# zhaodong-liu/GRAM

Measured on AMD Instinct MI355X. Metric: users/sec @ beam=20 top-20 gen, Beauty T5-base; Recall@5 parity, higher is better.
Workload: dtype f16x3

## Files before the change

### gram_amd/_lib.py

```python
from __future__ import annotations

import ctypes as C
import os

_HERE = os.path.dirname(os.path.abspath(__file__))
LIB_PATH = os.environ.get("GRAM_LIB") or os.path.join(_HERE, "csrc", "libgram_hip.so")

GRAM_MAX_BEAMS = 64
GRAM_MAX_DEC_LEN = 64
GRAM_MAX_PASSAGE_LEN = 128
GRAM_MAX_LONG_PASSAGE_LEN = 512
GRAM_MAX_FUSED_LEN = 4096
GRAM_MAX_LONG_FUSED_LEN = 16384
GRAM_KEY_BITS_LONG_WORDS, GRAM_KEY_BITS_LONG_STRIDE = 512, 528
EPI_BF16, EPI_BF16_RELU, EPI_F32_ADD, EPI_F32, EPI_KV_BANK = range(5)
K_GEMM, K_ENC_ATTN, K_CROSS_ATTN, K_DEC_SELF_ATTN, K_ROWOPS, K_LSE, K_BEAM = range(7)
E_ARG, E_WORKSPACE, E_BEAM, E_NONFINITE = -1, -2, -3, -4
ABI_VERSION = 7
GRAM_MAX_USER_ITEMS = 4096
ITEMS_EXCLUDE, ITEMS_ALLOW = 0, 1
MAX_PIECES = 2
SPLIT_NPROD = (0, 1, 3)


def interleave(pieces):
    p, rows, cols = pieces.shape
    assert p == 2 and cols % 32 == 0
    return pieces.view(2, rows, cols // 32, 32).permute(1, 2, 0, 3).reshape(rows, 2 * cols).contiguous()


def deinterleave(x):
    rows, c2 = x.shape
    return x.view(rows, c2 // 64, 2, 32).permute(2, 0, 1, 3).reshape(2, rows, c2 // 2).contiguous()


STAGES = ("enc_attn", "enc_ffn", "bank_k", "bank_v", "dec_self", "dec_cross", "dec_ffn", "lm_head")

vp = C.c_void_p
i32 = C.c_int32
i64 = C.c_int64
f32 = C.c_float


class KVBank(C.Structure):
    _fields_ = [("k", vp), ("vt", vp), ("n_layers", i32), ("B", i32), ("H", i32), ("S", i32), ("passage_map", vp), ("N", i32),
                ("L", i32)]


class Trie(C.Structure):
    _fields_ = [("child_off", vp), ("child_tok", vp), ("child_node", vp), ("n_nodes", i32), ("n_edges", i32),
                ("max_fanout", i32), ("min_seq_len", i32)]


class LiveRows(C.Structure):
    _fields_ = [("rows", vp), ("rowpos", vp), ("users", vp), ("tokens", vp), ("counts", vp)]


class BeamState(C.Structure):
    _fields_ = [("B", i32), ("K", i32), ("Tmax", i32), ("length_penalty", f32), ("eos", i32), ("pad", i32),
                ("tokens", vp), ("node", vp), ("beam_scores", vp), ("seq", vp), ("anc", vp), ("done", vp),
                ("n_hyps", vp), ("hyp_score", vp), ("worst", vp), ("hyp_len", vp), ("hyp_tok", vp), ("error", vp),
                ("cand_logits", vp), ("cand_logits_users", i32), ("cand_logits_stride", i64)]


class Split(C.Structure):
    _fields_ = [("pieces", i32), ("c_interleaved", i32), ("c_pstride", i64), ("bank_pstride", i64), ("out_scale", f32)]


class NormFusion(C.Structure):
    _fields_ = [("xb_out", vp), ("ss_out", vp), ("ss_in", vp), ("nblk_in", i32), ("d", i32), ("eps", f32), ("quarter", i32),
                ("xs_in", vp), ("xs_out", vp)]


class Compaction(C.Structure):
    _fields_ = [("n_active", i32), ("passage_map", vp), ("ids", vp), ("mask", vp),
                ("n_cached", i32), ("cache_L", i32), ("cache_x", vp), ("cache_slot", vp)]


class UserItems(C.Structure):
    _fields_ = [("leaf_lo", vp), ("leaf_hi", vp), ("ranks", vp), ("count", vp), ("stride", i32), ("mode", i32)]


class XattnOut(C.Structure):
    _fields_ = [("probs", vp), ("layer_probs", vp), ("token_scores", vp), ("passage_scores", vp)]


class TrieRows(C.Structure):
    _fields_ = [("tokens", vp), ("pos", vp), ("anc", vp), ("row_node", vp), ("node_row", vp), ("node_tok", vp), ("node_leaf", vp),
                ("Q", i32), ("Tq", i32), ("n_nodes", i32), ("n_leaves", i32)]


class ModelDesc(C.Structure):
    _fields_ = [
        ("vocab", i32), ("d_model", i32), ("d_ff", i32), ("n_heads", i32), ("n_enc_layers", i32),
        ("n_dec_layers", i32), ("max_passages", i32), ("tie_word_embeddings", i32),
        ("use_position_embedding", i32), ("fold_norm", i32), ("eps", f32),
        ("embed_f32", vp), ("lm_head_bf16", vp), ("pos_emb_f32", vp), ("enc_bias_f32", vp), ("dec_bias_f32", vp),
        ("enc_final_ln", vp), ("dec_final_ln", vp),
        ("enc_ln1", C.POINTER(vp)), ("enc_wqkv", C.POINTER(vp)), ("enc_wo", C.POINTER(vp)),
        ("enc_ln2", C.POINTER(vp)), ("enc_wi", C.POINTER(vp)), ("enc_wo2", C.POINTER(vp)),
        ("dec_ln1", C.POINTER(vp)), ("dec_wqkv", C.POINTER(vp)), ("dec_wo", C.POINTER(vp)),
        ("dec_ln2", C.POINTER(vp)), ("dec_wq_x", C.POINTER(vp)), ("dec_wo_x", C.POINTER(vp)),
        ("dec_ln3", C.POINTER(vp)), ("dec_wi", C.POINTER(vp)), ("dec_wo2", C.POINTER(vp)),
        ("dec_wkv_x_all", vp),
        ("pieces", i32), ("lm_head_f32", vp), ("w_scales", C.POINTER(f32)),
    ]


SIGNATURES = {
    "gram_abi_version": (C.c_int, []),
    "gram_piece_format": (C.c_int, []),
    "gram_gemm_bf16": (C.c_int, [vp, vp, vp, C.c_int, C.c_int, C.c_int, C.c_int, C.c_int, C.c_int, C.POINTER(KVBank), vp]),
    "gram_gemm_bf16_ex": (C.c_int, [vp, vp, vp, C.c_int, C.c_int, C.c_int, C.c_int, C.c_int, C.c_int, C.POINTER(KVBank), C.POINTER(NormFusion), vp]),
    "gram_row_rscale": (C.c_int, [vp, vp, C.c_int, C.c_int, C.c_int, f32, vp]),
    "gram_row_rscale_xs": (C.c_int, [vp, vp, vp, vp, C.c_int, C.c_int, C.c_int, f32, vp]),
    "gram_embed_ex_xs": (C.c_int, [vp, vp, C.c_int, vp, vp, vp, vp, C.c_int, C.c_int, C.c_int, C.c_int, vp]),
    "gram_embed_ex": (C.c_int, [vp, vp, C.c_int, vp, vp, vp, C.c_int, C.c_int, C.c_int, vp]),
    "gram_gemm_bf16_lse": (C.c_int, [vp, vp, vp, vp, C.c_int, C.c_int, C.c_int, C.c_int, C.c_int, vp]),
    "gram_lse_combine": (C.c_int, [vp, vp, C.c_int, C.c_int, vp]),
    "gram_embed_i64": (C.c_int, [vp, vp, vp, C.c_int, C.c_int, vp]),
    "gram_embed_i32": (C.c_int, [vp, vp, vp, C.c_int, C.c_int, vp]),
    "gram_rmsnorm_bf16": (C.c_int, [vp, vp, vp, C.c_int, C.c_int, f32, f32, vp, C.c_int, C.c_int, vp]),
    "gram_enc_self_attn": (C.c_int, [vp, vp, vp, vp, C.c_int, C.c_int, C.c_int, vp]),
    "gram_cross_attn_decode": (C.c_int, [vp, vp, vp, vp, vp, C.c_int, C.c_int, C.c_int, C.c_int, vp]),
    "gram_dec_self_attn": (C.c_int, [vp, vp, vp, vp, vp, vp, C.c_int, C.c_int, C.c_int, C.c_int, vp]),
    "gram_row_lse": (C.c_int, [vp, vp, C.c_int, C.c_int, vp]),
    "gram_beam_init": (C.c_int, [C.POINTER(BeamState), C.POINTER(Trie), C.c_int, vp]),
    "gram_beam_step": (C.c_int, [C.POINTER(BeamState), C.POINTER(Trie), vp, vp, C.c_int, C.c_int, C.c_int, vp]),
    "gram_beam_step_sparse": (C.c_int, [C.POINTER(BeamState), C.POINTER(Trie), vp, vp, C.c_int, vp, C.c_int, C.c_int, C.c_int, vp]),
    "gram_greedy_step": (C.c_int, [C.POINTER(BeamState), C.POINTER(Trie), vp, C.c_int, C.c_int, vp]),
    "gram_greedy_finalize": (C.c_int, [C.POINTER(BeamState), C.c_int, vp, vp, vp]),
    "gram_beam_finalize": (C.c_int, [C.POINTER(BeamState), C.c_int, C.c_int, vp, vp, vp, vp]),
    "gram_trie_item_index": (C.c_int, [C.POINTER(Trie), vp, vp, C.c_int, C.c_int, vp, vp]),
    "gram_model_create": (vp, [C.POINTER(ModelDesc)]),
    "gram_model_destroy": (None, [vp]),
    "gram_iota_i32": (C.c_int, [vp, C.c_int, vp]),
    "gram_token_tables_bytes": (i64, [vp]),
    "gram_token_tables_workspace_bytes": (i64, [vp]),
    "gram_model_build_token_tables": (C.c_int, [vp, vp, i64, vp, i64, vp]),
    "gram_workspace_bytes": (i64, [vp, C.c_int, C.c_int, C.c_int, C.c_int, C.c_int]),
    "gram_workspace_encoder_x_offset": (i64, [vp, C.c_int, C.c_int, C.c_int, C.c_int, C.c_int]),
    "gram_encode_fused": (C.c_int, [vp, vp, vp, C.c_int, C.c_int, C.c_int, vp, i64, C.c_int, C.c_int, vp, vp]),
# ... 20 lines not shown
                                              C.POINTER(UserItems), vp]),
    "gram_beam_step_sparse_split_items": (C.c_int, [C.POINTER(BeamState), C.POINTER(Trie), vp, vp, C.c_int, vp, C.c_int, C.c_int, C.c_int,
                                                    vp, C.c_int, C.POINTER(UserItems), vp]),
    "gram_greedy_step_items": (C.c_int, [C.POINTER(BeamState), C.POINTER(Trie), vp, C.c_int, C.c_int, C.POINTER(UserItems), vp]),
    "gram_generate_items": (C.c_int, [vp, vp, vp, C.c_int, C.c_int, C.c_int, C.c_int, C.c_int, C.c_int, f32, C.POINTER(Trie),
                                      C.POINTER(Compaction), C.POINTER(UserItems), vp, i64, vp, vp, C.POINTER(i32), vp]),
    "gram_encode_passages": (C.c_int, [vp, vp, vp, C.c_int, C.c_int, vp, i64, vp, vp]),
    "gram_gather_passage_x": (C.c_int, [vp, vp, vp, C.c_int, C.c_int, C.c_int, C.c_int, vp]),
    "gram_live_rows": (C.c_int, [C.POINTER(BeamState), C.POINTER(Trie), C.POINTER(LiveRows), vp]),
    "gram_dec_self_attn_live": (C.c_int, [vp, vp, vp, vp, vp, vp, C.c_int, C.c_int, vp, C.c_int, C.c_int, C.c_int, vp]),
    "gram_cross_attn_decode_live": (C.c_int, [vp, vp, vp, vp, vp, C.c_int, vp, vp, C.c_int, C.c_int, C.c_int, vp]),
    "gram_beam_step_sparse_live": (C.c_int, [C.POINTER(BeamState), C.POINTER(Trie), vp, vp, C.c_int, vp, C.c_int, C.c_int, vp, vp]),
    "gram_gemm_bf16_split": (C.c_int, [vp, vp, vp, C.c_int, C.c_int, C.c_int, C.c_int, C.c_int, C.c_int, C.POINTER(KVBank),
                                       C.POINTER(NormFusion), C.POINTER(Split), vp]),
    "gram_gemm_bf16_lse_split": (C.c_int, [vp, vp, vp, vp, C.c_int, C.c_int, C.c_int, C.c_int, C.c_int, C.POINTER(Split), vp]),
    "gram_embed_ex_split": (C.c_int, [vp, vp, C.c_int, vp, vp, vp, C.c_int, C.c_int, C.c_int, C.c_int, vp]),
    "gram_rmsnorm_bf16_split": (C.c_int, [vp, vp, vp, C.c_int, C.c_int, f32, f32, vp, C.c_int, C.c_int, vp, C.c_int, vp]),
    "gram_enc_self_attn_split": (C.c_int, [vp, vp, vp, vp, C.c_int, C.c_int, C.c_int, C.c_int, i64, vp]),
    "gram_cross_attn_decode_split": (C.c_int, [vp, vp, vp, vp, vp, C.c_int, C.c_int, C.c_int, C.c_int, vp, vp, C.c_int, i64, i64, vp, vp]),
    "gram_enc_self_attn_rows_split": (C.c_int, [vp, vp, vp, vp, vp, C.c_int, C.c_int, C.c_int, C.c_int, i64, vp]),
    "gram_enc_self_attn_long_split": (C.c_int, [vp, vp, vp, vp, C.c_int, C.c_int, C.c_int, C.c_int, i64, vp]),
    "gram_enc_self_attn_long_rows_split": (C.c_int, [vp, vp, vp, vp, vp, C.c_int, C.c_int, C.c_int, C.c_int, i64, vp]),
    "gram_model_set_max_passage_len": (C.c_int, [vp, C.c_int]),
    "gram_mask_key_bits": (C.c_int, [vp, vp, C.c_int, C.c_int, vp]),
    "gram_model_set_max_fused_len": (C.c_int, [vp, C.c_int]),
    "gram_mask_key_bits_long": (C.c_int, [vp, vp, C.c_int, C.c_int, vp]),
    "gram_cross_attn_long_scratch_bytes": (i64, [C.c_int, C.c_int, C.c_int]),
    "gram_cross_attn_long_split": (C.c_int, [vp, vp, vp, vp, vp, C.c_int, C.c_int, C.c_int, C.c_int, vp, vp, C.c_int, i64, i64, vp, vp, vp]),
    "gram_cross_attn_rows_long_split": (C.c_int, [vp, vp, vp, vp, vp, C.c_int, C.c_int, C.c_int, C.c_int, C.c_int, i64, i64, vp, vp, vp, vp]),
    "gram_dec_self_attn_split": (C.c_int, [vp, vp, vp, vp, vp, vp, C.c_int, C.c_int, vp, C.c_int, C.c_int, C.c_int, C.c_int, i64, i64, vp]),
    "gram_dec_self_attn_rows_split": (C.c_int, [vp, vp, vp, vp, vp, vp, vp, C.c_int, C.c_int, vp, C.c_int, C.c_int, C.c_int, C.c_int, i64, i64,
                                                vp]),
    "gram_beam_step_sparse_split": (C.c_int, [C.POINTER(BeamState), C.POINTER(Trie), vp, vp, C.c_int, vp, C.c_int, C.c_int, C.c_int,
                                              vp, C.c_int, vp]),
    "gram_generate": (C.c_int, [vp, vp, vp, C.c_int, C.c_int, C.c_int, C.c_int, C.c_int, C.c_int, f32, C.POINTER(Trie),
                                vp, i64, vp, vp, C.POINTER(i32), vp]),
    "gram_workspace_bytes_tf": (i64, [vp, C.c_int, C.c_int, C.c_int, C.c_int, C.c_int]),
    "gram_teacher_forced": (C.c_int, [vp, vp, vp, C.c_int, C.c_int, C.c_int, C.POINTER(Compaction), vp, vp, C.c_int, C.c_int, vp, i64,
                                      vp, vp, vp, vp]),
    "gram_dec_self_attn_tf_split": (C.c_int, [vp, vp, vp, C.c_int, C.c_int, C.c_int, C.c_int, i64, vp]),
    "gram_cross_attn_rows_split": (C.c_int, [vp, vp, vp, vp, vp, C.c_int, C.c_int, C.c_int, C.c_int, C.c_int, i64, i64, vp, vp, vp]),
    "gram_label_logprob_split": (C.c_int, [vp, vp, vp, C.c_int, vp, vp, C.c_int, C.c_int, C.c_int, C.c_int, vp, vp, vp]),
    "gram_cross_attn_probs_split": (C.c_int, [vp, vp, vp, vp, C.c_int, C.c_int, C.c_int, C.c_int, C.c_int, i64, i64, vp, vp]),
    "gram_xattn_head_sum": (C.c_int, [vp, vp, C.c_int, C.c_int, C.c_int, C.c_int, C.c_int, vp]),
    "gram_xattn_passage_scores": (C.c_int, [vp, vp, vp, C.c_int, C.c_int, C.c_int, C.c_int, f32, vp]),
    "gram_teacher_forced_ex": (C.c_int, [vp, vp, vp, C.c_int, C.c_int, C.c_int, C.POINTER(Compaction), vp, vp, C.c_int, C.c_int, vp, i64,
                                         vp, vp, vp, C.POINTER(XattnOut), vp]),
    "gram_dec_self_attn_tree_split": (C.c_int, [vp, vp, vp, vp, vp, C.c_int, C.c_int, C.c_int, C.c_int, C.c_int, i64, vp]),
    "gram_trie_repeat_tokens": (C.c_int, [vp, vp, C.c_int, C.c_int, vp]),
    "gram_trie_leaf_logprob_split": (C.c_int, [vp, vp, vp, C.c_int, vp, C.POINTER(TrieRows), C.c_int, C.c_int, C.c_int, vp, vp, vp, vp]),
    "gram_workspace_bytes_trie": (i64, [vp, C.c_int, C.c_int, C.c_int, C.c_int]),
    "gram_score_trie": (C.c_int, [vp, vp, vp, C.c_int, C.c_int, C.c_int, C.POINTER(Compaction), C.POINTER(Trie), C.POINTER(TrieRows), vp,
                                  i64, vp, vp, vp]),
}

for _old, _new in (("gram_gemm_bf16", "gram_gemm_f16"), ("gram_gemm_bf16_ex", "gram_gemm_f16_ex"), ("gram_gemm_bf16_split", "gram_gemm_f16_split"),
                   ("gram_gemm_bf16_lse", "gram_gemm_f16_lse"), ("gram_gemm_bf16_lse_split", "gram_gemm_f16_lse_split"),
                   ("gram_rmsnorm_bf16", "gram_rmsnorm_f16"), ("gram_rmsnorm_bf16_map", "gram_rmsnorm_f16_map"),
                   ("gram_rmsnorm_bf16_split", "gram_rmsnorm_f16_split")):
    SIGNATURES[_new] = SIGNATURES[_old]

_lib = None


def load() -> C.CDLL:
    global _lib
    if _lib is not None:
        return _lib
    import torch
    if not os.path.exists(LIB_PATH):
        raise ImportError(
            f"{LIB_PATH} not found: the HIP extension is not built (run __graft_entry__.build() or "
            "`make -C gram_amd/csrc`).  gram_amd has no CPU fallback."
        )
    lib = C.CDLL(LIB_PATH)
    for name, (res, args) in SIGNATURES.items():
        fn = getattr(lib, name)
        fn.restype = res
        fn.argtypes = args
    if lib.gram_abi_version() != ABI_VERSION:
        raise ImportError("libgram_hip.so ABI version mismatch")
    _lib = lib
    return lib


class GramHipError(RuntimeError):
    pass


def piece_dtype():
    import torch
    return torch.float16 if load().gram_piece_format() == 1 else torch.bfloat16


def check(code: int, what: str) -> None:
    if code == 0:
        return
    names = {E_ARG: "GRAM_E_ARG (bad shape / unsupported size)", E_WORKSPACE: "GRAM_E_WORKSPACE",
             E_BEAM: "GRAM_E_BEAM (impossible beam state; HF would raise here)",
             E_NONFINITE: "GRAM_E_NONFINITE (a returned score is NaN / +inf: an activation left the range of the 16-bit pieces -- IEEE half, "
                          "|x| <= 65504; build and load the bfloat16 library: make -C gram_amd/csrc PIECE=bf16, GRAM_LIB=.../libgram_hip_bf16.so)"}
    raise GramHipError(f"{what} failed: {names.get(code, f'hipError {code}')}")
```

### gram_amd/csrc/beam.hip

```cpp
#include <stdlib.h>

#include "common.h"
#include "prof.h"
#include "sparse_dot.h"

namespace {

__device__ __forceinline__ uint32_t f2ord(float f) {
  uint32_t u = __float_as_uint(f);
  return (u & 0x80000000u) ? ~u : (u | 0x80000000u);
}
__device__ __forceinline__ float ord2f(uint32_t o) {
  uint32_t u = (o & 0x80000000u) ? (o & 0x7fffffffu) : ~o;
  return __uint_as_float(u);
}

__device__ int find_child(const gram_trie_t& tr, int node, int tok) {
  if (node < 0) return -1;
  int lo = tr.child_off[node], hi = tr.child_off[node + 1];
  while (lo < hi) {
    int mid = (lo + hi) >> 1;
    int v = tr.child_tok[mid];
    if (v == tok) return mid;
    if (v < tok) lo = mid + 1; else hi = mid;
// ... 898 lines not shown
  for (int i = tid * per; i < (tid + 1) * per; ++i) c += keep(i) ? 1 : 0;
  s_cnt[tid] = c;
  gram_sync();
  if (tid == 0) {
    int acc = 0;
    for (int t = 0; t < 256; ++t) {
      const int n = s_cnt[t];
      s_cnt[t] = acc;
      acc += n;
    }
    count[b] = acc < stride ? acc : stride;
  }
  gram_sync();
  int pos = s_cnt[tid];
  for (int i = tid * per; i < (tid + 1) * per; ++i)
    if (keep(i)) {
      if (pos < stride) ranks[(size_t)b * stride + pos] = s[i];
      ++pos;
    }
}

__global__ void greedy_finalize_kernel(gram_beam_state_t st, int max_length, int64_t* __restrict__ sequences,
                                       int32_t* __restrict__ out_width) {
  const int b = blockIdx.x * blockDim.x + threadIdx.x;
  if (b >= st.B) return;
  const int T = st.Tmax;
  for (int p = 0; p < max_length; ++p) sequences[(size_t)b * max_length + p] = st.seq[(size_t)b * T + p];
  const int len = st.n_hyps[b] > 0 ? st.n_hyps[b] : max_length;
  atomicMax(out_width, len);
}

__global__ void trie_item_index_kernel(gram_trie_t tr, const int32_t* __restrict__ node_item, const int64_t* __restrict__ sequences,
                                       int rows, int T, int pad, int32_t* __restrict__ out_item) {
  const int r = blockIdx.x * blockDim.x + threadIdx.x;
  if (r >= rows) return;
  const int64_t* seq = sequences + (size_t)r * T;
  int node = 0, p = 0;
  for (; p < T; ++p) {
    if (tr.child_off[node + 1] == tr.child_off[node]) break;
    const int64_t tok = seq[p];
    const int e = (tok < 0 || tok > 0x7fffffff) ? -1 : find_child(tr, node, (int)tok);
    if (e < 0) { node = -1; break; }
    node = tr.child_node[e];
  }
  int item = -1;
  if (node > 0 && tr.child_off[node + 1] == tr.child_off[node]) {
    item = node_item[node];
    for (; p < T; ++p)
      if (seq[p] != pad) item = -1;
  }
  out_item[r] = item;
}

}

static int check_state(const gram_beam_state_t* st) {
  if (!st || st->B < 1 || st->K < 1 || st->K > GRAM_MAX_BEAMS || st->Tmax < 2 || st->Tmax > GRAM_MAX_DEC_LEN) return GRAM_E_ARG;
  return 0;
}

extern "C" int gram_beam_init(const gram_beam_state_t* st, const gram_trie_t* tr, int start_token, void* stream) {
  if (int e = check_state(st)) return e;
  if (!tr) return GRAM_E_ARG;
  const int R = st->B * st->K;
  hipLaunchKernelGGL(beam_init_kernel, dim3((R + 255) / 256), dim3(256), 0, (hipStream_t)stream, *st, *tr, start_token);
  GRAM_CHECK_LAUNCH();
  return 0;
}

static int g_beam_chunked = -1;
static int g_beam_chunk_cap = 0;
extern "C" int gram_debug_set_beam_chunked(int mode) {
  if (mode < -1 || mode > 1) return GRAM_E_ARG;
  g_beam_chunked = mode;
  return 0;
}
extern "C" int gram_debug_set_beam_chunk_capacity(int candidates) {
  if (candidates < 0) return GRAM_E_ARG;
  g_beam_chunk_cap = candidates;
  return 0;
}

static int check_items(const gram_user_items_t* it) {
  if (!it || !it->leaf_lo || !it->leaf_hi || !it->ranks || !it->count || it->stride < 1 || it->stride > GRAM_MAX_USER_ITEMS ||
      (it->mode != GRAM_ITEMS_EXCLUDE && it->mode != GRAM_ITEMS_ALLOW))
    return GRAM_E_ARG;
  return 0;
}

static int launch_beam_step(const gram_beam_state_t* st, const gram_trie_t* tr, const float* logits, const float* lse, int V,
                            int cur_len, int rows_per_user, const void* hd, const void* emb, int d, const int32_t* rowpos,
                            void* stream, int pieces = 1, const float* emb32 = nullptr, const gram_user_items_t* items = nullptr) {
  if (int e = check_state(st)) return e;
  if (!tr || !lse || cur_len < 1 || cur_len >= st->Tmax || V < 2 || (rows_per_user != 1 && rows_per_user != st->K)) return GRAM_E_ARG;
  if (!logits && (!hd || (!emb && !emb32) || d < 64 || (d & 63))) return GRAM_E_ARG;
  if (pieces < 1 || pieces > GRAM_MAX_PIECES || (pieces > 1 && (!emb32 || (d & 63)))) return GRAM_E_ARG;
  if (tr->max_fanout < 0) return GRAM_E_ARG;
  long long need = (long long)st->K * tr->max_fanout;
  int nc = 64;
  while (nc < need && nc < kOneShotMaxKeys) nc <<= 1;
  const size_t seq_bytes = (size_t)2 * st->K * st->Tmax * 4;
  const size_t smem_one = (size_t)nc * 8 + ((size_t)tr->max_fanout * 4 + 15) / 16 * 16 + seq_bytes;
  const bool chunked = g_beam_chunked == 1 || need > kOneShotMaxKeys || smem_one > 152 * 1024;
  gram_prof::Scope prof(GRAM_K_BEAM, (hipStream_t)stream, 0.0);
  static const int wide_max_b = getenv("GRAM_BEAM_WIDE_MAXB") ? atoi(getenv("GRAM_BEAM_WIDE_MAXB")) : 128;
  if (chunked) {
// ... 107 lines not shown
extern "C" int gram_beam_step_sparse_live(const gram_beam_state_t* st, const gram_trie_t* tr, const void* hidden_bf16,
                                          const void* lm_head_bf16, int d, const float* lse, int V, int cur_len,
                                          const int32_t* rowpos, void* stream) {
  if (!rowpos || !st) return GRAM_E_ARG;
  return launch_beam_step(st, tr, nullptr, lse, V, cur_len, st->K, hidden_bf16, lm_head_bf16, d, rowpos, stream);
}

extern "C" int gram_beam_step_sparse_split(const gram_beam_state_t* st, const gram_trie_t* tr, const void* hidden_bf16,
                                           const float* lm_head_f32, int d, const float* lse, int V, int cur_len, int rows_per_user,
                                           const int32_t* rowpos, int pieces, void* stream) {
  if (!lm_head_f32) return GRAM_E_ARG;
  return launch_beam_step(st, tr, nullptr, lse, V, cur_len, rows_per_user, hidden_bf16, nullptr, d, rowpos, stream, pieces, lm_head_f32);
}

extern "C" int gram_beam_step_sparse_items(const gram_beam_state_t* st, const gram_trie_t* tr, const void* hidden_bf16,
                                           const void* lm_head_bf16, int d, const float* lse, int V, int cur_len, int rows_per_user,
                                           const int32_t* rowpos, const gram_user_items_t* items, void* stream) {
  if (int e = check_items(items)) return e;
  if (!st || (rowpos && rows_per_user != st->K)) return GRAM_E_ARG;
  return launch_beam_step(st, tr, nullptr, lse, V, cur_len, rows_per_user, hidden_bf16, lm_head_bf16, d, rowpos, stream, 1, nullptr, items);
}

extern "C" int gram_beam_step_sparse_split_items(const gram_beam_state_t* st, const gram_trie_t* tr, const void* hidden_bf16,
                                                 const float* lm_head_f32, int d, const float* lse, int V, int cur_len,
                                                 int rows_per_user, const int32_t* rowpos, int pieces, const gram_user_items_t* items,
                                                 void* stream) {
  if (int e = check_items(items)) return e;
  if (!lm_head_f32 || !st || (rowpos && rows_per_user != st->K)) return GRAM_E_ARG;
  return launch_beam_step(st, tr, nullptr, lse, V, cur_len, rows_per_user, hidden_bf16, nullptr, d, rowpos, stream, pieces, lm_head_f32,
                          items);
}

extern "C" int gram_user_items_prepare(const int32_t* item_rank, int n_items, const int32_t* items, int B, int M, int32_t* ranks,
                                       int32_t* count, int stride, void* stream) {
  if (!item_rank || !items || !ranks || !count || n_items < 1 || B < 1 || M < 1 || stride < M || stride > GRAM_MAX_USER_ITEMS)
    return GRAM_E_ARG;
  int npad = 256;
  while (npad < M) npad <<= 1;
  hipLaunchKernelGGL(user_items_prepare_kernel, dim3(B), dim3(256), (size_t)npad * 4, (hipStream_t)stream, item_rank, n_items, items, M,
                     npad, ranks, count, stride);
  GRAM_CHECK_LAUNCH();
  return 0;
}

extern "C" int gram_live_rows(const gram_beam_state_t* st, const gram_trie_t* tr, const gram_live_rows_t* out, void* stream) {
  if (int e = check_state(st)) return e;
  if (!tr || !out || !out->rows || !out->rowpos || !out->users || !out->tokens || !out->counts) return GRAM_E_ARG;
  gram_prof::Scope prof(GRAM_K_BEAM, (hipStream_t)stream, 0.0);
  hipLaunchKernelGGL(live_rows_kernel, dim3(1), dim3(1024), 0, (hipStream_t)stream, *st, *tr, *out);
  GRAM_CHECK_LAUNCH();
  return 0;
}

extern "C" int gram_greedy_step(const gram_beam_state_t* st, const gram_trie_t* tr, const float* logits, int V, int cur_len,
                               void* stream) {
  if (int e = check_state(st)) return e;
  if (!tr || st->K != 1 || cur_len < 1 || cur_len >= st->Tmax || V < 2) return GRAM_E_ARG;
  gram_prof::Scope prof(GRAM_K_BEAM, (hipStream_t)stream, 0.0);
  hipLaunchKernelGGL(greedy_step_kernel, dim3((st->B + 127) / 128), dim3(128), 0, (hipStream_t)stream, *st, *tr, logits, V, cur_len);
  GRAM_CHECK_LAUNCH();
  return 0;
}

extern "C" int gram_greedy_step_items(const gram_beam_state_t* st, const gram_trie_t* tr, const float* logits, int V, int cur_len,
                                      const gram_user_items_t* items, void* stream) {
  if (int e = check_items(items)) return e;
  if (int e = check_state(st)) return e;
  if (!tr || st->K != 1 || cur_len < 1 || cur_len >= st->Tmax || V < 2) return GRAM_E_ARG;
  gram_prof::Scope prof(GRAM_K_BEAM, (hipStream_t)stream, 0.0);
  hipLaunchKernelGGL(greedy_step_items_kernel, dim3((st->B + 127) / 128), dim3(128), 0, (hipStream_t)stream, *st, *tr, logits, V, cur_len,
                     *items);
  GRAM_CHECK_LAUNCH();
  return 0;
}

extern "C" int gram_greedy_finalize(const gram_beam_state_t* st, int max_length, int64_t* sequences, int32_t* out_width,
                                    void* stream) {
  if (int e = check_state(st)) return e;
  if (st->K != 1 || max_length != st->Tmax) return GRAM_E_ARG;
  hipError_t e = hipMemsetAsync(out_width, 0, sizeof(int32_t), (hipStream_t)stream);
  if (e != hipSuccess) return (int)e;
  hipLaunchKernelGGL(greedy_finalize_kernel, dim3((st->B + 127) / 128), dim3(128), 0, (hipStream_t)stream, *st, max_length, sequences,
                     out_width);
  GRAM_CHECK_LAUNCH();
  return 0;
}

extern "C" int gram_beam_finalize(const gram_beam_state_t* st, int nret, int max_length, int64_t* sequences, float* scores,
                                  int32_t* out_width, void* stream) {
  if (int e = check_state(st)) return e;
  if (nret < 1 || nret > st->K || max_length != st->Tmax) return GRAM_E_ARG;
  hipError_t e = hipMemsetAsync(out_width, 0, sizeof(int32_t), (hipStream_t)stream);
  if (e != hipSuccess) return (int)e;
  hipLaunchKernelGGL(beam_finalize_kernel, dim3(st->B), dim3(64), 0, (hipStream_t)stream, *st, nret, max_length, max_length,
                     sequences, scores, out_width);
  GRAM_CHECK_LAUNCH();
  return 0;
}

extern "C" int gram_trie_item_index(const gram_trie_t* tr, const int32_t* node_item, const int64_t* sequences, int rows, int T,
                                    int32_t* out_item, void* stream) {
  if (!tr || !tr->child_off || !node_item || !sequences || !out_item || rows < 0 || T < 1 || tr->n_nodes < 1) return GRAM_E_ARG;
  if (rows == 0) return 0;
  hipLaunchKernelGGL(trie_item_index_kernel, dim3((rows + 255) / 256), dim3(256), 0, (hipStream_t)stream, *tr, node_item, sequences, rows,
                     T, 0, out_item);
  GRAM_CHECK_LAUNCH();
// ... 3 lines not shown
```

### gram_amd/csrc/dec_attn.hip

```cpp
#include <type_traits>

#include "common.h"
#include "prof.h"
#include "xattn_tile.h"

namespace {

__device__ __forceinline__ void xa_merge_w(float m0, float m1, float l0, float l1, float& w0, float& w1, float& inv) {
  const float M = fmaxf(fmaxf(GRAM_FMIN, m0), m1);
  w0 = __expf(m0 - M);
  w1 = __expf(m1 - M);
  inv = 1.f / __builtin_fmaf(l1, w1, l0 * w0);
}
__device__ __forceinline__ f32x4 xa_merge_o(f32x4 o0, f32x4 o1, float w0, float w1, float inv) {
  f32x4 r;
#pragma unroll
  for (int e = 0; e < 4; ++e) r[e] = __builtin_fmaf(o1[e], w1, o0[e] * w0) * inv;
  return r;
}

template <int NT, bool LIVE, int S, int NW>
__global__ __launch_bounds__(NW * 64) void cross_attn_kernel(
    const p16* __restrict__ q, const p16* __restrict__ kbank, const p16* __restrict__ vtbank,
    const uint8_t* __restrict__ mask, p16* __restrict__ out, int K, int H, int Sk, const int32_t* __restrict__ users,
    const int32_t* __restrict__ rowpos, long q_pstride, long bank_pstride, const uint32_t* __restrict__ key_bits) {
  using T = SplitTab<S>;
  constexpr int NB = NT * 16;
  static_assert(NW == 1 || NW == 2, "the merge is written for two waves");
  constexpr int PSTR = 2 * XA_TILE;
  constexpr int STAGE = S * PSTR;
  extern __shared__ __attribute__((aligned(16))) char smem[];
  float* sm_m = reinterpret_cast<float*>(smem);
  float* sm_l = sm_m + NW * NB;
  float* sm_o = sm_l + NW * NB;

  const int h = blockIdx.x, b = LIVE ? users[blockIdx.y] : blockIdx.y;
  const int tid = threadIdx.x, lane = tid & 63;
  const int wave = __builtin_amdgcn_readfirstlane(tid >> 6);
  const int c = lane & 15, g = lane >> 4;
  const int inner = H * 64;
  const char* kb = reinterpret_cast<const char*>(kbank + ((size_t)b * H + h) * Sk * 64);
  const char* vt = reinterpret_cast<const char*>(vtbank + ((size_t)b * H + h) * 64 * Sk);
  const uint8_t* mk = mask + (size_t)b * Sk;

  p16x8 qf[S][NT][2];
  f32x4 o[4][NT];
  float m[NT], l[NT];
#pragma unroll
  for (int nt = 0; nt < NT; ++nt) {
    m[nt] = GRAM_FMIN;
    l[nt] = 0.f;
#pragma unroll
    for (int mt = 0; mt < 4; ++mt) o[mt][nt] = (f32x4){0.f, 0.f, 0.f, 0.f};
  }

#pragma unroll
  for (int nt = 0; nt < NT; ++nt) {
    const int qrow = xa_row<LIVE>(b, K, 16 * nt + c, rowpos);
#pragma unroll
    for (int pc = 0; pc < S; ++pc)
#pragma unroll
      for (int kd = 0; kd < 2; ++kd)
        qf[pc][nt][kd] = qrow >= 0 ? ld_global_b128(q + pc * q_pstride + (size_t)qrow * inner + h * 64 + 32 * kd + 8 * g) : zero_bf16x8();
  }
  const int nsteps = Sk >> 5;
  uint32_t kb0 = 0, kb1 = 0;
  if (key_bits) {
    if (lane < nsteps) kb0 = key_bits[(size_t)b * 128 + lane];
    if (lane + 64 < nsteps) kb1 = key_bits[(size_t)b * 128 + 64 + lane];
  } else {
#pragma unroll
    for (int half = 0; half < 2; ++half) {
      const int st = lane + 64 * half;
      uint32_t bits = 0;
      if (st < nsteps) {
        const uint4* p = reinterpret_cast<const uint4*>(mk + 32 * st);
        const uint4 a = p[0], c2 = p[1];
        const uint32_t w8[8] = {a.x, a.y, a.z, a.w, c2.x, c2.y, c2.z, c2.w};
#pragma unroll
        for (int i = 0; i < 8; ++i)
#pragma unroll
          for (int j = 0; j < 4; ++j) bits |= ((w8[i] >> (8 * j)) & 0xffu) ? (1u << (4 * i + j)) : 0u;
      }
      if (half == 0) kb0 = bits; else kb1 = bits;
    }
  }
  unsigned long long v0 = __ballot(kb0 != 0u), v1 = __ballot(kb1 != 0u);
  if ((v0 | v1) == 0ull) {
    v0 = nsteps >= 64 ? ~0ull : ((1ull << nsteps) - 1ull);
    v1 = nsteps > 64 ? ((nsteps >= 128 ? ~0ull : ((1ull << (nsteps - 64)) - 1ull))) : 0ull;
  }
  v0 = __builtin_amdgcn_readfirstlane((unsigned)v0) | ((unsigned long long)__builtin_amdgcn_readfirstlane((unsigned)(v0 >> 32)) << 32);
  v1 = __builtin_amdgcn_readfirstlane((unsigned)v1) | ((unsigned long long)__builtin_amdgcn_readfirstlane((unsigned)(v1 >> 32)) << 32);
  int ord = 0;
  auto next = [&](int s) -> int {
    for (s = s + 1; s < nsteps; ++s) {
      const unsigned long long bit = (s < 64 ? (v0 >> s) : (v1 >> (s - 64))) & 1ull;
      if (bit) {
        const bool mine = ord == wave;
        ord = ord + 1 == NW ? 0 : ord + 1;
        if (mine) return s;
      }
    }
    return nsteps;
  };

  uint32_t koff[4], voff[4];
#pragma unroll
  for (int i = 0; i < 4; ++i) {
    const int kr = 8 * i + (lane >> 3);
    koff[i] = (uint32_t)(kr * 128 + (((lane & 7) ^ ksw(kr)) << 4));
// ... 86 lines not shown
      l[nt] = xa_l_update(l[nt], alpha, ps);
#pragma unroll
      for (int mt = 0; mt < 4; ++mt) o[mt][nt] *= alpha;
    }
  };
  auto math_pv = [&]() {
#pragma unroll
    for (int mt = 0; mt < 4; ++mt)
#pragma unroll
      for (int nt = 0; nt < NT; ++nt)
#pragma unroll
        for (int pr = 0; pr < T::NP; ++pr) o[mt][nt] = mfma16(vf[T::A[pr]][mt], pf[T::B[pr]][nt], o[mt][nt]);
  };

  wait_vm<0>();
#pragma unroll
  for (int nt = 0; nt < NT; ++nt)
#pragma unroll
    for (int pc = 0; pc < S; ++pc)
#pragma unroll
      for (int kd = 0; kd < 2; ++kd) asm volatile("" : "+v"(qf[pc][nt][kd]));
  int cur = next(-1);
  if (cur < nsteps) {
    issue_k(cur);
    issue_v(cur);
  }
  while (cur < nsteps) {
    const int nxt = next(cur);
    wait_vm<4 * S>();
    read_k();
    if (nxt < nsteps) {
      asm volatile("s_waitcnt lgkmcnt(0)" ::: "memory");
      issue_k(nxt);
    }
    math_qk(cur);
    if (nxt < nsteps) wait_vm<4 * S>();
    else wait_vm<0>();
    read_v();
    if (nxt < nsteps) {
      asm volatile("s_waitcnt lgkmcnt(0)" ::: "memory");
      issue_v(nxt);
    }
    math_pv();
    cur = nxt;
  }

  if constexpr (NW == 1) {
#pragma unroll
    for (int nt = 0; nt < NT; ++nt) {
      float lt = l[nt];
      lt += __shfl_xor(lt, 16, 64);
      lt += __shfl_xor(lt, 32, 64);
      const float inv = 1.f / lt;
      const int orow = xa_row<LIVE>(b, K, 16 * nt + c, rowpos);
      if (orow >= 0) {
#pragma unroll
        for (int mt = 0; mt < 4; ++mt) xa_store<S>(out, orow, inner, h * 64 + 16 * mt + 4 * g, o[mt][nt] * inv);
      }
    }
    return;
  }
  gram_sync();
#pragma unroll
  for (int nt = 0; nt < NT; ++nt) {
    float lt = l[nt];
    lt += __shfl_xor(lt, 16, 64);
    lt += __shfl_xor(lt, 32, 64);
    const int beam = 16 * nt + c;
    if (g == 0) {
      sm_m[wave * NB + beam] = m[nt];
      sm_l[wave * NB + beam] = lt;
    }
#pragma unroll
    for (int mt = 0; mt < 4; ++mt)
      *reinterpret_cast<f32x4*>(sm_o + ((size_t)(wave * NB + beam)) * 64 + 16 * mt + 4 * g) = o[mt][nt];
  }
  gram_sync();
  for (int idx = tid; idx < K * 16; idx += NW * 64) {
    const int beam = idx >> 4, d4 = (idx & 15) * 4;
    float w0, w1, inv2;
    xa_merge_w(sm_m[beam], sm_m[NB + beam], sm_l[beam], sm_l[NB + beam], w0, w1, inv2);
    const f32x4 v = xa_merge_o(*reinterpret_cast<const f32x4*>(sm_o + ((size_t)beam) * 64 + d4),
                         *reinterpret_cast<const f32x4*>(sm_o + ((size_t)(NB + beam)) * 64 + d4), w0, w1, inv2);
    int orow = b * K + beam;
    if constexpr (LIVE) orow = rowpos[orow];
    if (orow >= 0) xa_store<S>(out, orow, inner, h * 64 + d4, v);
  }
}

struct XaLaunch {
  const void *q, *k, *vt;
  const uint8_t* mask;
  void* out;
  int B, K, H, Sk;
  const int32_t *users, *rowpos;
  long q_ps, bank_ps;
  const uint32_t* key_bits;
  hipStream_t st;
};

template <int NT, int S>
int launch_cross(const XaLaunch& a) {
  constexpr int NW = NT >= 3 ? 1 : 2;
  constexpr int NB = NT * 16;
  constexpr int stages = NW * S * 2 * XA_TILE, merge = NW == 1 ? 0 : (2 * NW * NB + NW * NB * 64) * 4;
  constexpr int smem = stages > merge ? stages : merge;
  static_assert(smem <= 160 * 1024, "the stages do not fit the LDS");
  static bool attr_set = false;
  if (!attr_set) {
    hipError_t e = hipFuncSetAttribute(reinterpret_cast<const void*>(cross_attn_kernel<NT, false, S, NW>),
                                       hipFuncAttributeMaxDynamicSharedMemorySize, smem);
    if (e == hipSuccess)
      e = hipFuncSetAttribute(reinterpret_cast<const void*>(cross_attn_kernel<NT, true, S, NW>),
                              hipFuncAttributeMaxDynamicSharedMemorySize, smem);
    if (e != hipSuccess) return (int)e;
    attr_set = true;
  }
  if (a.users)
    hipLaunchKernelGGL((cross_attn_kernel<NT, true, S, NW>), dim3(a.H, a.B), dim3(NW * 64), smem, a.st, (const p16*)a.q, (const p16*)a.k,
                       (const p16*)a.vt, a.mask, (p16*)a.out, a.K, a.H, a.Sk, a.users, a.rowpos, a.q_ps, a.bank_ps, a.key_bits);
  else
    hipLaunchKernelGGL((cross_attn_kernel<NT, false, S, NW>), dim3(a.H, a.B), dim3(NW * 64), smem, a.st, (const p16*)a.q, (const p16*)a.k,
                       (const p16*)a.vt, a.mask, (p16*)a.out, a.K, a.H, a.Sk, a.users, a.rowpos, a.q_ps, a.bank_ps, a.key_bits);
  GRAM_CHECK_LAUNCH();
  return 0;
}

template <int S>
int launch_cross_nt(const XaLaunch& a) {
  switch ((a.K + 15) / 16) {
    case 1: return launch_cross<1, S>(a);
    case 2: return launch_cross<2, S>(a);
    case 3: return launch_cross<3, S>(a);
    default: return launch_cross<4, S>(a);
  }
}

__global__ __launch_bounds__(128) void mask_key_bits_kernel(const uint8_t* __restrict__ mask, uint32_t* __restrict__ bits, int Sk) {
  const int b = blockIdx.x, st = threadIdx.x;
  uint32_t w = 0;
  if (st < (Sk >> 5)) {
    const uint4* p = reinterpret_cast<const uint4*>(mask + (size_t)b * Sk + 32 * st);
    const uint4 a = p[0], c2 = p[1];
    const uint32_t w8[8] = {a.x, a.y, a.z, a.w, c2.x, c2.y, c2.z, c2.w};
#pragma unroll
    for (int i = 0; i < 8; ++i)
#pragma unroll
      for (int j = 0; j < 4; ++j) w |= ((w8[i] >> (8 * j)) & 0xffu) ? (1u << (4 * i + j)) : 0u;
  }
  bits[(size_t)b * 128 + st] = w;
}

template <int S>
__global__ __launch_bounds__(256) void dec_self_attn_kernel(const p16* __restrict__ qkv, p16* __restrict__ kcache,
                                                            p16* __restrict__ vcache, const int32_t* __restrict__ anc,
                                                            const float* __restrict__ bias, p16* __restrict__ out, int R,
                                                            int H, int t, const int32_t* __restrict__ rows, long qkv_ps,
                                                            long cache_ps, const int32_t* __restrict__ qkv_rows) {
  const int rc = blockIdx.x, i = threadIdx.x;
  const int r = rows ? rows[rc] : rc;
  const int inner = H * 64, h = i >> 4;
  const p16* row = qkv + (size_t)(qkv_rows ? qkv_rows[rc] : rc) * 3 * inner + 4 * i;
  float qf[4] = {0.f, 0.f, 0.f, 0.f}, kn[4] = {0.f, 0.f, 0.f, 0.f}, vn[4] = {0.f, 0.f, 0.f, 0.f};
#pragma unroll
  for (int pc = S - 1; pc >= 0; --pc) {
    const p16x4 q4 = *reinterpret_cast<const p16x4*>(row + pc * qkv_ps);
    const p16x4 k4 = *reinterpret_cast<const p16x4*>(row + pc * qkv_ps + inner);
    const p16x4 v4 = *reinterpret_cast<const p16x4*>(row + pc * qkv_ps + 2 * inner);
    *reinterpret_cast<p16x4*>(kcache + pc * cache_ps + ((size_t)t * R + r) * inner + 4 * i) = k4;
    *reinterpret_cast<p16x4*>(vcache + pc * cache_ps + ((size_t)t * R + r) * inner + 4 * i) = v4;
#pragma unroll
    for (int e = 0; e < 4; ++e) {
      qf[e] += (float)q4[e];
      kn[e] += (float)k4[e];
      vn[e] += (float)v4[e];
    }
  }
  float m = -INFINITY, l = 0.f, acc[4] = {0.f, 0.f, 0.f, 0.f};
  auto attend = [&](int j, const float (&kj)[4], const float (&vj)[4]) {
    float s = qf[0] * kj[0] + qf[1] * kj[1] + qf[2] * kj[2] + qf[3] * kj[3];
    s += __shfl_xor(s, 1, 64);
    s += __shfl_xor(s, 2, 64);
    s += __shfl_xor(s, 4, 64);
    s += __shfl_xor(s, 8, 64);
    s += bias[h * GRAM_MAX_DEC_LEN + (t - j)];
    const float mn = fmaxf(m, s);
    const float alpha = __expf(m - mn);
    const float p = __expf(s - mn);
    m = mn;
    l = l * alpha + p;
#pragma unroll
    for (int e = 0; e < 4; ++e) acc[e] = acc[e] * alpha + p * vj[e];
  };
  constexpr int U = 8;
  for (int j0 = 0; j0 < t; j0 += U) {
    int a[U];
#pragma unroll
    for (int u = 0; u < U; ++u) a[u] = anc[(size_t)min(j0 + u, t - 1) * R + r];
    p16x4 kk[U][S], vv[U][S];
#pragma unroll
    for (int u = 0; u < U; ++u) {
      const size_t off = ((size_t)min(j0 + u, t - 1) * R + a[u]) * inner + 4 * i;
#pragma unroll
      for (int pc = 0; pc < S; ++pc) {
        kk[u][pc] = ld_stream_b64(kcache + pc * cache_ps + off);
        vv[u][pc] = ld_stream_b64(vcache + pc * cache_ps + off);
      }
    }
#pragma unroll
    for (int u = 0; u < U; ++u) {
      if (j0 + u < t) {
        float kj[4] = {0.f, 0.f, 0.f, 0.f}, vj[4] = {0.f, 0.f, 0.f, 0.f};
#pragma unroll
        for (int pc = S - 1; pc >= 0; --pc)
#pragma unroll
          for (int e = 0; e < 4; ++e) {
            kj[e] += (float)kk[u][pc][e];
            vj[e] += (float)vv[u][pc][e];
          }
        attend(j0 + u, kj, vj);
      }
    }
  }
  attend(t, kn, vn);
  const float inv = 1.f / l;
#pragma unroll
  for (int e = 0; e < 4; ++e) acc[e] *= inv;
#pragma unroll
  for (int pc = 0; pc < S; ++pc) {
    p16x4 o;
#pragma unroll
    for (int e = 0; e < 4; ++e) {
      o[e] = (p16)acc[e];
      acc[e] -= (float)o[e];
    }
    *reinterpret_cast<p16x4*>(out + (size_t)rc * inner * S + (S == 2 ? inter_off(4 * i, pc) : 4 * i)) = o;
  }
}

}

extern "C" int gram_mask_key_bits(const uint8_t* mask, uint32_t* key_bits, int B, int S, void* stream) {
  if (!mask || !key_bits || B < 1 || S < 32 || (S & 31) || S > 4096 || (reinterpret_cast<uintptr_t>(mask) & 15)) return GRAM_E_ARG;
  hipLaunchKernelGGL(mask_key_bits_kernel, dim3(B), dim3(128), 0, (hipStream_t)stream, mask, key_bits, S);
  GRAM_CHECK_LAUNCH();
  return 0;
}

extern "C" int gram_cross_attn_decode_split(const void* q, const void* k_layer, const void* vt_layer, const uint8_t* mask, void* out,
                                            int B, int K, int H, int S, const int32_t* users, const int32_t* rowpos, int pieces,
                                            int64_t q_pstride, int64_t bank_pstride, const uint32_t* key_bits, void* stream) {
  if (B < 1 || K < 1 || K > GRAM_MAX_BEAMS || H < 1 || S < 32 || (S & 31) || S > 4096 || pieces < 1 || pieces > GRAM_MAX_PIECES ||
      (users == nullptr) != (rowpos == nullptr))
    return GRAM_E_ARG;
  if (pieces > 1 && (q_pstride < 1 || bank_pstride < (int64_t)H * S * 64)) return GRAM_E_ARG;
  if ((reinterpret_cast<uintptr_t>(mask) & 15) || (reinterpret_cast<uintptr_t>(k_layer) & 15) || (reinterpret_cast<uintptr_t>(vt_layer) & 15))
    return GRAM_E_ARG;
  hipStream_t st = (hipStream_t)stream;
  gram_prof::Scope prof(GRAM_K_CROSS_ATTN, st, 4.0 * B * H * S * 64 * pieces);
  const XaLaunch a{q, k_layer, vt_layer, mask, out, B, K, H, S, users, rowpos, (long)q_pstride, (long)bank_pstride, key_bits, st};
  return pieces == 2 ? launch_cross_nt<2>(a) : launch_cross_nt<1>(a);
}

extern "C" int gram_cross_attn_decode(const void* q, const void* k_layer, const void* vt_layer, const uint8_t* mask, void* out,
                                      int B, int K, int H, int S, void* stream) {
  return gram_cross_attn_decode_split(q, k_layer, vt_layer, mask, out, B, K, H, S, nullptr, nullptr, 1, 0, 0, nullptr, stream);
}

extern "C" int gram_cross_attn_decode_live(const void* q, const void* k_layer, const void* vt_layer, const uint8_t* mask, void* out,
                                           int n_users, const int32_t* users, const int32_t* rowpos, int K, int H, int S,
                                           void* stream) {
  if (!users || !rowpos) return GRAM_E_ARG;
  return gram_cross_attn_decode_split(q, k_layer, vt_layer, mask, out, n_users, K, H, S, users, rowpos, 1, 0, 0, nullptr, stream);
}

extern "C" int gram_dec_self_attn_split(const void* qkv, void* kcache, void* vcache, const int32_t* anc, const float* bias, void* out,
                                        int R, int n_rows, const int32_t* rows, int H, int t, int Tmax, int pieces,
                                        int64_t qkv_pstride, int64_t cache_pstride, void* stream) {
  return gram_dec_self_attn_rows_split(qkv, nullptr, kcache, vcache, anc, bias, out, R, n_rows, rows, H, t, Tmax, pieces, qkv_pstride,
                                       cache_pstride, stream);
}

extern "C" int gram_dec_self_attn_rows_split(const void* qkv, const int32_t* qkv_rows, void* kcache, void* vcache, const int32_t* anc,
                                             const float* bias, void* out, int R, int n_rows, const int32_t* rows, int H, int t,
                                             int Tmax, int pieces, int64_t qkv_pstride, int64_t cache_pstride, void* stream) {
  if (R < 1 || n_rows < 1 || n_rows > R || H < 1 || H > 16 || t < 0 || t >= Tmax || Tmax > GRAM_MAX_DEC_LEN || pieces < 1 ||
      pieces > GRAM_MAX_PIECES)
    return GRAM_E_ARG;
  if (pieces > 1 && (qkv_pstride < 1 || cache_pstride < (int64_t)Tmax * R * H * 64)) return GRAM_E_ARG;
  hipStream_t st = (hipStream_t)stream;
  gram_prof::Scope prof(GRAM_K_DEC_SELF_ATTN, st, 4.0 * n_rows * H * 64 * (t + 1) * pieces);
  const dim3 grid(n_rows), block(H * 16);
// ... 21 lines not shown
```

### gram_amd/csrc/generate.hip

```cpp
#include <stdlib.h>
#include <string.h>
#include <vector>

#include "common.h"
#include "prof.h"

struct gram_model {
  gram_model_desc_t d;
  std::vector<const float*> enc_ln1, enc_ln2, dec_ln1, dec_ln2, dec_ln3;
  std::vector<const void*> enc_wqkv, enc_wo, enc_wi, enc_wo2, dec_wqkv, dec_wo, dec_wq_x, dec_wo_x, dec_wi, dec_wo2;
  std::vector<float> s_enc_wqkv, s_enc_wo, s_enc_wi, s_enc_wo2, s_dec_wqkv, s_dec_wo, s_dec_wq_x, s_dec_wo_x, s_dec_wi, s_dec_wo2;
  float s_wkv = 1.f, s_lm = 1.f;
  const p16 *enc_qkv0 = nullptr, *dec_qkv0 = nullptr;
  int max_L = GRAM_MAX_PASSAGE_LEN;
  int max_S = GRAM_MAX_FUSED_LEN;
  bool long_xattn() const { return max_S > GRAM_MAX_FUSED_LEN; }
};

namespace {

struct Carve {
  char* base;
  int64_t off;
  explicit Carve(void* p) : base((char*)p), off(0) {}
  template <typename T>
  T* take(int64_t n) {
    off = (off + 255) & ~(int64_t)255;
    T* p = base ? reinterpret_cast<T*>(base + off) : nullptr;
    off += n * (int64_t)sizeof(T);
    return p;
  }
};

constexpr int64_t kStreamRowsLimit = GRAM_STREAM_MAX_M_LIMIT;
inline int64_t ss_floats(int64_t rows, int64_t d) {
  const int64_t q = (rows < kStreamRowsLimit ? rows : kStreamRowsLimit) * (d / 16), full = rows * (d / 64);
  return q > full ? q : full;
}
struct Rows {
  float* x;
  p16* h;
  p16* qkv;
  p16* attn;
  p16* qx;
  p16* u;
  float* ss;
  float* rs;
  float* xs[2];
  int64_t ps_qkv, ps_qx;
};
struct Workspace {
  Rows enc, dec;
  p16* bank_k;
  p16* bank_vt;
  p16* kcache;
  p16* vcache;
  float* logits;
  float* lse;
  float* lse_part;
  gram_beam_state_t beam;
  gram_live_rows_t live;
  int32_t* width;
  uint32_t* key_bits;
  float* xa_scratch;
  int32_t* rowmap;
  int64_t bytes;
  int pieces;
  int64_t ps_bank, ps_cache;
};

Rows take_rows(Carve& cv, const gram_model_desc_t& c, int64_t P, int64_t rows, bool decoder) {
  const int64_t d = c.d_model, inner = (int64_t)c.n_heads * 64;
  Rows r{};
  r.ps_qkv = rows * 3 * inner;
  r.ps_qx = rows * inner;
  r.x = cv.take<float>(rows * d);
  r.h = cv.take<p16>(P * rows * d);
  r.qkv = cv.take<p16>(P * r.ps_qkv);
  r.attn = cv.take<p16>(P * rows * inner);
  if (decoder) r.qx = cv.take<p16>(P * r.ps_qx);
  r.u = cv.take<p16>(P * rows * c.d_ff);
  r.ss = cv.take<float>(ss_floats(rows, d));
  r.rs = cv.take<float>(rows);
  r.xs[0] = cv.take<float>(rows);
  r.xs[1] = cv.take<float>(rows);
  return r;
}
void take_key_bits(Carve& cv, Workspace& w, const gram_model* m, int64_t B, int64_t rows, int S) {
  if (!m->long_xattn()) {
    w.key_bits = cv.take<uint32_t>(B * 128);
    return;
  }
  w.key_bits = cv.take<uint32_t>(B * GRAM_KEY_BITS_LONG_STRIDE);
  const int64_t n = gram_cross_attn_long_scratch_bytes((int)rows, m->d.n_heads, S) / (int64_t)sizeof(float);
  w.xa_scratch = n > 0 ? cv.take<float>(n) : nullptr;
}
void take_bank(Carve& cv, Workspace& w, const gram_model_desc_t& c, int64_t B, int64_t S) {
  w.ps_bank = c.n_dec_layers * B * c.n_heads * S * 64;
  w.bank_k = cv.take<p16>(w.pieces * w.ps_bank);
  w.bank_vt = cv.take<p16>(w.pieces * w.ps_bank);
}

Workspace carve(const gram_model* m, void* ws, int B, int N, int L, int K, int Tmax) {
  const gram_model_desc_t& c = m->d;
  const int64_t inner = (int64_t)c.n_heads * 64, V = c.vocab, R = (int64_t)B * K, nl = c.n_dec_layers;
  Carve cv(ws);
  Workspace w{};
  const int64_t P = w.pieces = c.pieces > 1 ? c.pieces : 1;
  w.enc = take_rows(cv, c, P, (int64_t)B * N * L, false);
  take_bank(cv, w, c, B, (int64_t)N * L);
  w.dec = take_rows(cv, c, P, R, true);
  w.ps_cache = nl * Tmax * R * inner;
  w.kcache = cv.take<p16>(P * w.ps_cache);
  w.vcache = cv.take<p16>(P * w.ps_cache);
  w.logits = cv.take<float>(R * V);
  w.lse = cv.take<float>(R);
  w.lse_part = cv.take<float>(R * (V / 64) * 2);
  gram_beam_state_t& s = w.beam;
  s.B = B;
  s.K = K;
  s.Tmax = Tmax;
  s.length_penalty = 1.f;
  s.eos = 1;
  s.pad = 0;
  s.tokens = cv.take<int32_t>(R);
  s.node = cv.take<int32_t>(R);
  s.beam_scores = cv.take<float>(R);
  s.seq = cv.take<int32_t>(R * Tmax);
  s.anc = cv.take<int32_t>((int64_t)Tmax * R);
  s.done = cv.take<int32_t>(B);
  s.n_hyps = cv.take<int32_t>(B);
  s.hyp_score = cv.take<double>((int64_t)B * (K + 1));
  s.worst = cv.take<double>(B);
  s.hyp_len = cv.take<int32_t>((int64_t)B * (K + 1));
  s.hyp_tok = cv.take<int32_t>((int64_t)B * (K + 1) * Tmax);
  s.error = cv.take<int32_t>(4);
  s.cand_logits_users = B < 16 ? B : 16;
  s.cand_logits_stride = 16384;
  s.cand_logits = cv.take<float>((int64_t)s.cand_logits_users * s.cand_logits_stride);
  w.live.rows = cv.take<int32_t>(R);
  w.live.rowpos = cv.take<int32_t>(R);
  w.live.users = cv.take<int32_t>(B);
  w.live.tokens = cv.take<int32_t>(R);
  w.live.counts = cv.take<int32_t>(4);
  w.width = cv.take<int32_t>(4);
  take_key_bits(cv, w, m, B, R, N * L);
  w.bytes = (cv.off + 255) & ~(int64_t)255;
  return w;
}

int check_shapes(const gram_model* m, int B, int N, int L, int K, int Tmax) {
  if (!m || B < 1 || N < 1 || N > m->d.max_passages || L < 32 || L > m->max_L || (L & 31) || N * L > m->max_S || K < 1 ||
      K > GRAM_MAX_BEAMS || Tmax < 2 || Tmax > GRAM_MAX_DEC_LEN)
    return GRAM_E_ARG;
  return 0;
}

constexpr int kPrecomputedRsRows = 32768;

#define TRY(x)            \
  do {                    \
    int e__ = (x);        \
    if (e__) return e__;  \
  } while (0)

int g_stage_cap[GRAM_STAGE_COUNT] = {99, 99, 99, 99, 99, 99, 99, 99};
int cap_planar(const Workspace& w, void* buf, int64_t ps, int stage, void* st) {
  if (w.pieces < 2 || g_stage_cap[stage] >= 2) return 0;
  hipError_t e = hipMemsetAsync((p16*)buf + (size_t)ps, 0, (size_t)ps * sizeof(p16), (hipStream_t)st);
  return e == hipSuccess ? 0 : (int)e;
}
int cap_inter(const Workspace& w, void* buf, int64_t rows, int64_t cols, int stage, void* st) {
  if (w.pieces < 2 || g_stage_cap[stage] >= 2) return 0;
  hipError_t e = hipMemset2DAsync((char*)buf + 64, 128, 0, 64, (size_t)(rows * cols / 32), (hipStream_t)st);
  return e == hipSuccess ? 0 : (int)e;
}

enum { C_NONE = 0, C_PLANAR = 1, C_INTER = 2 };
int linear(const Workspace& w, const void* A, const void* W, float out_scale, void* C, int c_kind, int64_t c_ps, int M, int N, int kc, int epi,
           const gram_kv_bank_t* bank, const gram_norm_fusion_t* nf, void* st) {
  const int P = w.pieces;
  const gram_split_t sp{P, c_kind == C_INTER, c_ps, w.ps_bank, out_scale};
  return gram_gemm_bf16_split(A, W, C, M, N, kc, P * kc, c_kind == C_INTER ? P * N : N, epi, bank, nf, &sp, st);
}

struct NormChain {
  const gram_model_desc_t& c;
  const Workspace& w;
  const Rows& r;
  const int n, d;
  void* const st;
  const int quarter;
  const bool pre_rs;
  int np = 0;

  NormChain(const gram_model* m, const Workspace& w, const Rows& r, int n, void* st)
      : c(m->d), w(w), r(r), n(n), d(c.d_model), st(st),
        quarter(c.fold_norm && n <= gram_gemm_stream_max_m() && d % 128 == 0 && (c.n_heads * 64) % 128 == 0 && c.d_ff % 128 == 0),
        pre_rs(n >= kPrecomputedRsRows) {}

  int embed(const void* ids, int ids_are_i64, bool want_xb = true) {
    if (c.fold_norm)
      return gram_embed_ex_xs(c.embed_f32, ids, ids_are_i64, r.x, want_xb ? r.h : nullptr, r.ss, r.xs[0], d / 64, n, d, w.pieces, st);
// ... 180 lines not shown
  return gram_gemm_bf16_split(w.dec.h, c.lm_head_bf16, logits, n, V, d, w.pieces * d, V, GRAM_EPI_F32, nullptr, nullptr, &sp, st);
}

int decode_step(const gram_model* m, const Workspace& w, const int32_t* tokens, const int32_t* anc, const uint8_t* mask, int B,
                int N, int L, int K, int R_cache, int Tmax, int t, float* logits, float* lse_part, const LiveStep* live,
                void* st) {
  const gram_model_desc_t& c = m->d;
  const int inner = c.n_heads * 64, H = c.n_heads;
  const int R = live ? live->n_rows : B * K, S = N * L;
  const size_t bank_layer = (size_t)B * H * S * 64;
  const size_t cache_layer = (size_t)Tmax * R_cache * inner;
  const Rows& r = w.dec;
  const p16* const table = token_table(m, m->dec_qkv0, GRAM_STAGE_DEC_SELF);
  TRY(decoder_layers(
      m, w, tokens, R, table != nullptr,
      [&](int i) {
        if (i == 0 && table)
          return gram_dec_self_attn_rows_split(table, tokens, w.kcache, w.vcache, anc, c.dec_bias_f32, r.attn, live ? R_cache : R, R,
                                               live ? live->rows : nullptr, H, t, Tmax, w.pieces, (int64_t)c.vocab * 3 * inner,
                                               w.ps_cache, st);
        return gram_dec_self_attn_split(r.qkv, w.kcache + i * cache_layer, w.vcache + i * cache_layer, anc, c.dec_bias_f32, r.attn,
                                        live ? R_cache : R, R, live ? live->rows : nullptr, H, t, Tmax, w.pieces, r.ps_qkv, w.ps_cache, st);
      },
      [&](int i) {
        if (m->long_xattn())
          return gram_cross_attn_long_split(r.qx, w.bank_k + i * bank_layer, w.bank_vt + i * bank_layer, mask, r.attn,
                                            live ? live->n_users : B, K, H, S, live ? live->users : nullptr,
                                            live ? live->rowpos : nullptr, w.pieces, r.ps_qx, w.ps_bank, w.key_bits, w.xa_scratch, st);
        return gram_cross_attn_decode_split(r.qx, w.bank_k + i * bank_layer, w.bank_vt + i * bank_layer, mask, r.attn,
                                            live ? live->n_users : B, K, H, S, live ? live->users : nullptr, live ? live->rowpos : nullptr,
                                            w.pieces, r.ps_qx, w.ps_bank, w.key_bits, st);
      },
      st));
  return lm_head(m, w, R, logits, lse_part, st);
}

int search_step(const gram_model* m, const Workspace& w, const gram_trie_t* trie, int cur_len, int rows_per_user, const int32_t* rowpos,
                const gram_user_items_t* items, void* st) {
  const gram_model_desc_t& c = m->d;
  if (items) {
    if (w.pieces > 1)
      return gram_beam_step_sparse_split_items(&w.beam, trie, w.dec.h, c.lm_head_f32, c.d_model, w.lse, c.vocab, cur_len, rows_per_user,
                                               rowpos, w.pieces, items, st);
    return gram_beam_step_sparse_items(&w.beam, trie, w.dec.h, c.lm_head_bf16, c.d_model, w.lse, c.vocab, cur_len, rows_per_user, rowpos,
                                       items, st);
  }
  if (w.pieces > 1)
    return gram_beam_step_sparse_split(&w.beam, trie, w.dec.h, c.lm_head_f32, c.d_model, w.lse, c.vocab, cur_len, rows_per_user, rowpos,
                                       w.pieces, st);
  if (rowpos) return gram_beam_step_sparse_live(&w.beam, trie, w.dec.h, c.lm_head_bf16, c.d_model, w.lse, c.vocab, cur_len, rowpos, st);
  return gram_beam_step_sparse(&w.beam, trie, w.dec.h, c.lm_head_bf16, c.d_model, w.lse, c.vocab, cur_len, rows_per_user, st);
}

}

extern "C" int gram_abi_version(void) { return GRAM_ABI_VERSION; }
extern "C" int gram_piece_format(void) { return GRAM_PIECE_FORMAT; }

extern "C" int gram_debug_set_stage_pieces(const int32_t* caps, int n) {
  if (caps && n != GRAM_STAGE_COUNT) return GRAM_E_ARG;
  for (int i = 0; i < GRAM_STAGE_COUNT; ++i) g_stage_cap[i] = caps ? (caps[i] < 1 ? 1 : caps[i]) : 99;
  return 0;
}

static int g_live_rows = -1;
extern "C" int gram_debug_set_live_rows(int on) {
  g_live_rows = on;
  return 0;
}
extern "C" int gram_debug_set_token_tables(int on) {
  g_token_tables = on;
  return 0;
}

extern "C" gram_model_t* gram_model_create(const gram_model_desc_t* d) {
  if (!d || d->vocab < 128 || d->d_model < 128 || d->d_ff < 128 || d->vocab % 128 || d->d_model % 128 || d->d_ff % 128 ||
      d->n_heads < 1 || d->n_heads > 16 ||
      (d->n_heads * 64) % 128 || d->d_model > 1024 || d->n_enc_layers < 1 || d->n_dec_layers < 1)
    return nullptr;
  if (d->pieces < 0 || d->pieces > GRAM_MAX_PIECES || (d->pieces > 1 && (!d->lm_head_f32 || !d->fold_norm))) return nullptr;
  gram_model* m = new gram_model();
  m->d = *d;
  auto own = [](auto& v, auto& p, int n) {
    v.assign(p, p + n);
    p = v.data();
  };
  gram_model_desc_t& c = m->d;
  own(m->enc_ln1, c.enc_ln1, c.n_enc_layers);
  own(m->enc_ln2, c.enc_ln2, c.n_enc_layers);
  own(m->enc_wqkv, c.enc_wqkv, c.n_enc_layers);
  own(m->enc_wo, c.enc_wo, c.n_enc_layers);
  own(m->enc_wi, c.enc_wi, c.n_enc_layers);
  own(m->enc_wo2, c.enc_wo2, c.n_enc_layers);
  own(m->dec_ln1, c.dec_ln1, c.n_dec_layers);
  own(m->dec_ln2, c.dec_ln2, c.n_dec_layers);
  own(m->dec_ln3, c.dec_ln3, c.n_dec_layers);
  own(m->dec_wqkv, c.dec_wqkv, c.n_dec_layers);
  own(m->dec_wo, c.dec_wo, c.n_dec_layers);
  own(m->dec_wq_x, c.dec_wq_x, c.n_dec_layers);
  own(m->dec_wo_x, c.dec_wo_x, c.n_dec_layers);
  own(m->dec_wi, c.dec_wi, c.n_dec_layers);
  own(m->dec_wo2, c.dec_wo2, c.n_dec_layers);
  {
    const float* ws = d->w_scales;
    auto take = [&](std::vector<float>& v, int n) {
      v.assign(n, 1.f);
// ... 112 lines not shown
extern "C" int64_t gram_workspace_encoder_x_offset(const gram_model_t* m, int B, int N, int L, int K, int max_length) {
  if (check_shapes(m, B, N, L, K, max_length)) return GRAM_E_ARG;
  const Workspace w = carve(m, (void*)256, B, N, L, K, max_length);
  return (int64_t)((const char*)w.enc.x - (const char*)256);
}

extern "C" int gram_encode_fused(const gram_model_t* m, const int64_t* input_ids, const uint8_t* mask, int B, int N, int L,
                                 void* workspace, int64_t workspace_bytes, int K, int max_length, void* enc_out_bf16,
                                 void* stream) {
  TRY(check_shapes(m, B, N, L, K, max_length));
  Workspace w = carve(m, workspace, B, N, L, K, max_length);
  if (!workspace || workspace_bytes < w.bytes) return GRAM_E_WORKSPACE;
  TRY(encode_call(m, w, input_ids, mask, B, N, L, nullptr, stream));
  if (enc_out_bf16) {
    hipError_t e = hipMemcpyAsync(enc_out_bf16, w.enc.h, (size_t)w.pieces * B * N * L * m->d.d_model * sizeof(p16), hipMemcpyDeviceToDevice,
                                  (hipStream_t)stream);
    if (e != hipSuccess) return (int)e;
  }
  return 0;
}

extern "C" int gram_encode_passages(const gram_model_t* m, const int64_t* ids, const uint8_t* mask, int P, int L, void* workspace,
                                    int64_t workspace_bytes, float* x_out, void* stream) {
  TRY(check_shapes(m, P, 1, L, 1, 2));
  if (!ids || !mask || !x_out) return GRAM_E_ARG;
  Workspace w = carve(m, workspace, P, 1, L, 1, 2);
  if (!workspace || workspace_bytes < w.bytes) return GRAM_E_WORKSPACE;
  TRY(encoder_layers(m, w, ids, mask, L, P, stream));
  hipError_t e = hipMemcpyAsync(x_out, w.enc.x, (size_t)P * L * m->d.d_model * sizeof(float), hipMemcpyDeviceToDevice,
                                (hipStream_t)stream);
  return e == hipSuccess ? 0 : (int)e;
}

extern "C" int gram_decode_step(const gram_model_t* m, const int32_t* tokens, const int32_t* anc, const uint8_t* mask, int B, int N,
                                int L, int K, int max_length, int t, void* workspace, int64_t workspace_bytes, float* logits,
                                void* stream) {
  TRY(check_shapes(m, B, N, L, K, max_length));
  if (t < 0 || t >= max_length - 1 || !logits) return GRAM_E_ARG;
  Workspace w = carve(m, workspace, B, N, L, K, max_length);
  if (!workspace || workspace_bytes < w.bytes) return GRAM_E_WORKSPACE;
  return decode_step(m, w, tokens, anc, mask, B, N, L, K, B * K, max_length, t, logits, nullptr, nullptr, stream);
}

extern "C" int gram_generate(const gram_model_t* m, const int64_t* input_ids, const uint8_t* mask, int B, int N, int L, int K,
                             int nret, int max_length, float length_penalty, const gram_trie_t* trie, void* workspace,
                             int64_t workspace_bytes, int64_t* sequences, float* scores, int32_t* width_host, void* stream) {
  return gram_generate_ex(m, input_ids, mask, B, N, L, K, nret, max_length, length_penalty, trie, nullptr, workspace, workspace_bytes,
                          sequences, scores, width_host, stream);
}

namespace {
int generate_body(const gram_model* m, Workspace& w, const int64_t* input_ids, const uint8_t* mask, int B, int N, int L, int K, int nret,
                  int max_length, const gram_trie_t* trie, const gram_compaction_t* comp, const gram_user_items_t* items,
                  int64_t* sequences, float* scores, void* stream) {
  TRY(encode_call(m, w, input_ids, mask, B, N, L, comp, stream));
  TRY(gram_beam_init(&w.beam, trie, 0, stream));
  if (K == 1) {
    for (int t = 0; t + 1 < max_length; ++t) {
      TRY(decode_step(m, w, w.beam.tokens, w.beam.anc, mask, B, N, L, 1, B, max_length, t, w.logits, nullptr, nullptr, stream));
      if (items) TRY(gram_greedy_step_items(&w.beam, trie, w.logits, m->d.vocab, t + 1, items, stream));
      else TRY(gram_greedy_step(&w.beam, trie, w.logits, m->d.vocab, t + 1, stream));
    }
    TRY(gram_greedy_finalize(&w.beam, max_length, sequences, w.width, stream));
  } else {
    static const bool live_rows_env = [] {
      const char* e = getenv("GRAM_LIVE_ROWS");
      return !(e && e[0] == '0');
    }();
    const bool live_rows = g_live_rows < 0 ? live_rows_env : g_live_rows != 0;
    for (int t = 0; t + 1 < max_length; ++t) {
      const int Kt = t == 0 ? 1 : K;
      if (live_rows && t >= 1 && trie->min_seq_len >= 2 && t >= trie->min_seq_len - 1) {
        int32_t counts[2] = {0, 0};
        TRY(gram_live_rows(&w.beam, trie, &w.live, stream));
        hipError_t e = hipMemcpyAsync(counts, w.live.counts, sizeof(counts), hipMemcpyDeviceToHost, (hipStream_t)stream);
        if (e == hipSuccess) e = hipStreamSynchronize((hipStream_t)stream);
        if (e != hipSuccess) return (int)e;
        if (counts[0] < 0 || counts[0] > B * K || counts[1] < 0 || counts[1] > B) return GRAM_E_BEAM;
        if (counts[0] < B * K) {
          if (counts[0] > 0) {
            const LiveStep live{counts[0], counts[1], w.live.rows, w.live.rowpos, w.live.users};
            TRY(decode_step(m, w, w.live.tokens, w.beam.anc, mask, B, N, L, K, B * K, max_length, t, nullptr, w.lse_part, &live,
                            stream));
            TRY(gram_lse_combine(w.lse_part, w.lse, counts[0], m->d.vocab / 64, stream));
          }
          TRY(search_step(m, w, trie, t + 1, K, w.live.rowpos, items, stream));
          continue;
        }
      }
      TRY(decode_step(m, w, w.beam.tokens, w.beam.anc, mask, B, N, L, Kt, B * K, max_length, t, nullptr, w.lse_part, nullptr,
                      stream));
      TRY(gram_lse_combine(w.lse_part, w.lse, B * Kt, m->d.vocab / 64, stream));
      TRY(search_step(m, w, trie, t + 1, Kt, nullptr, items, stream));
    }
    TRY(gram_beam_finalize(&w.beam, nret, max_length, sequences, scores, w.width, stream));
  }
  return 0;
}

}

static int generate_call(const gram_model_t* m, const int64_t* input_ids, const uint8_t* mask, int B, int N, int L, int K, int nret,
                         int max_length, float length_penalty, const gram_trie_t* trie, const gram_compaction_t* comp,
                         const gram_user_items_t* items, void* workspace, int64_t workspace_bytes, int64_t* sequences, float* scores,
                         int32_t* width_host, void* stream) {
  TRY(check_shapes(m, B, N, L, K, max_length));
  TRY(check_compaction(comp, B, N));
  if (!trie || nret < 1 || nret > K || !sequences || (!scores && K != 1)) return GRAM_E_ARG;
  Workspace w = carve(m, workspace, B, N, L, K, max_length);
  if (!workspace || workspace_bytes < w.bytes) return GRAM_E_WORKSPACE;
  w.beam.length_penalty = length_penalty;
  TRY(generate_body(m, w, input_ids, mask, B, N, L, K, nret, max_length, trie, comp, items, sequences, scores, stream));
  if (width_host) {
    int32_t host[2] = {0, 0};
    hipError_t e = hipMemcpyAsync(&host[0], w.width, sizeof(int32_t), hipMemcpyDeviceToHost, (hipStream_t)stream);
    if (e == hipSuccess) e = hipMemcpyAsync(&host[1], w.beam.error, sizeof(int32_t), hipMemcpyDeviceToHost, (hipStream_t)stream);
    if (e == hipSuccess) e = hipStreamSynchronize((hipStream_t)stream);
    if (e != hipSuccess) return (int)e;
    *width_host = host[0];
    if (host[1] == 4) return GRAM_E_NONFINITE;
    if (host[1] != 0) return GRAM_E_BEAM;
  }
  return 0;
}

extern "C" int gram_generate_ex(const gram_model_t* m, const int64_t* input_ids, const uint8_t* mask, int B, int N, int L, int K,
                                int nret, int max_length, float length_penalty, const gram_trie_t* trie,
                                const gram_compaction_t* comp, void* workspace, int64_t workspace_bytes, int64_t* sequences,
                                float* scores, int32_t* width_host, void* stream) {
  return generate_call(m, input_ids, mask, B, N, L, K, nret, max_length, length_penalty, trie, comp, nullptr, workspace, workspace_bytes,
                       sequences, scores, width_host, stream);
}

extern "C" int gram_generate_items(const gram_model_t* m, const int64_t* input_ids, const uint8_t* mask, int B, int N, int L, int K,
                                   int nret, int max_length, float length_penalty, const gram_trie_t* trie,
                                   const gram_compaction_t* comp, const gram_user_items_t* items, void* workspace,
                                   int64_t workspace_bytes, int64_t* sequences, float* scores, int32_t* width_host, void* stream) {
  if (!items || !items->leaf_lo || !items->leaf_hi || !items->ranks || !items->count || items->stride < 1 ||
      items->stride > GRAM_MAX_USER_ITEMS || (items->mode != GRAM_ITEMS_EXCLUDE && items->mode != GRAM_ITEMS_ALLOW))
    return GRAM_E_ARG;
  return generate_call(m, input_ids, mask, B, N, L, K, nret, max_length, length_penalty, trie, comp, items, workspace, workspace_bytes,
                       sequences, scores, width_host, stream);
}

namespace {

int check_shapes_tf(const gram_model* m, int B, int N, int L, int C, int T) {
  if (!m || B < 1 || N < 1 || N > m->d.max_passages || L < 32 || L > m->max_L || (L & 31) || N * L > m->max_S || C < 1 ||
      T < 1 || T > GRAM_MAX_DEC_LEN || (int64_t)B * C * T > INT32_MAX / 4)
    return GRAM_E_ARG;
  return 0;
}

Workspace carve_tf(const gram_model* m, void* ws, int B, int N, int L, int C, int T) {
  const gram_model_desc_t& c = m->d;
  const int64_t V = c.vocab, R = (int64_t)B * C * T;
  Carve cv(ws);
  Workspace w{};
  const int64_t P = w.pieces = c.pieces > 1 ? c.pieces : 1;
  take_key_bits(cv, w, m, B, (int64_t)B * ((int64_t)C * T < GRAM_MAX_BEAMS ? C * T : GRAM_MAX_BEAMS), N * L);
  w.rowmap = cv.take<int32_t>((int64_t)B * (1 + 2 * GRAM_MAX_BEAMS));
  take_bank(cv, w, c, B, (int64_t)N * L);
  const int64_t shared = cv.off;
  w.enc = take_rows(cv, c, P, (int64_t)B * N * L, false);
  const int64_t enc_end = cv.off;
  cv.off = shared;
  w.dec = take_rows(cv, c, P, R, true);
  w.lse = cv.take<float>(R);
  w.lse_part = cv.take<float>(R * (V / 64) * 2);
  const int64_t end = cv.off > enc_end ? cv.off : enc_end;
  w.bytes = (end + 255) & ~(int64_t)255;
  return w;
}

int decoder_tf(const gram_model* m, const Workspace& w, const int32_t* tokens, const uint8_t* mask, int B, int N, int L, int Q, int T,
               float* logits, const gram_xattn_out_t* attn, const gram_trie_rows_t* tree, void* st) {
  const gram_model_desc_t& c = m->d;
  const int H = c.n_heads, R = B * Q, S = N * L;
  const size_t bank_layer = (size_t)B * H * S * 64;
  const Rows& r = w.dec;
  TRY(decoder_layers(
      m, w, tokens, R, false,
      [&](int) {
        if (tree)
          return gram_dec_self_attn_tree_split(r.qkv, tree->pos, tree->anc, c.dec_bias_f32, r.attn, B, Q, tree->Tq, H, w.pieces, r.ps_qkv,
                                               st);
        return gram_dec_self_attn_tf_split(r.qkv, c.dec_bias_f32, r.attn, R / T, T, H, w.pieces, r.ps_qkv, st);
      },
      [&](int i) {
        if (m->long_xattn())
          TRY(gram_cross_attn_rows_long_split(r.qx, w.bank_k + i * bank_layer, w.bank_vt + i * bank_layer, mask, r.attn, B, Q, H, S,
                                              w.pieces, r.ps_qx, w.ps_bank, w.key_bits, w.xa_scratch, w.rowmap, st));
        else
          TRY(gram_cross_attn_rows_split(r.qx, w.bank_k + i * bank_layer, w.bank_vt + i * bank_layer, mask, r.attn, B, Q, H, S, w.pieces,
                                         r.ps_qx, w.ps_bank, w.key_bits, w.rowmap, st));
// ... 94 lines not shown
```

### gram_amd/model/gram.py

```python
from __future__ import annotations

import ctypes as C
import math
import os
from typing import Callable, Dict, Optional

import torch
from torch import nn

from .. import _lib
from ..utils.generation_trie import FlatTrie, Trie


class GenerateOutput(dict):

    __getattr__ = dict.get


class ForwardOutput(dict):

    __getattr__ = dict.get

    def to_tuple(self):
        return tuple(v for v in (self.get("loss"), self.get("logits")) if v is not None)
# ... 66 lines not shown
        self.max_seq_len = getattr(c, "max_seq_len", 128)
        self.max_item_num = getattr(c, "max_item_num", 20)
        self.use_position_embedding = bool(getattr(c, "use_position_embedding", True))
        d, inner, F, V = c.d_model, c.num_heads * c.d_kv, c.d_ff, c.vocab_size
        self.model_dim = d
        dec_layers = c.num_decoder_layers if getattr(c, "num_decoder_layers", None) is not None else c.num_layers
        self._n_enc, self._n_dec = c.num_layers, dec_layers

        def P(*shape):
            return nn.Parameter(torch.empty(*shape, dtype=torch.float32))

        shared = P(V, d)
        _register(self, "shared.weight", shared)
        _register(self, "encoder.encoder.embed_tokens.weight", shared)
        _register(self, "decoder.embed_tokens.weight", shared)

        def attn(prefix, rel):
            _register(self, prefix + ".q.weight", P(inner, d))
            _register(self, prefix + ".k.weight", P(inner, d))
            _register(self, prefix + ".v.weight", P(inner, d))
            _register(self, prefix + ".o.weight", P(d, inner))
            if rel:
                _register(self, prefix + ".relative_attention_bias.weight", P(c.relative_attention_num_buckets, c.num_heads))

        def ff(prefix):
            _register(self, prefix + ".DenseReluDense.wi.weight", P(F, d))
            _register(self, prefix + ".DenseReluDense.wo.weight", P(d, F))

        for i in range(self._n_enc):
            p = f"encoder.encoder.block.{i}.module.layer"
            attn(p + ".0.SelfAttention", i == 0)
            _register(self, p + ".0.layer_norm.weight", P(d))
            ff(p + ".1")
            _register(self, p + ".1.layer_norm.weight", P(d))
        _register(self, "encoder.encoder.final_layer_norm.weight", P(d))
        for i in range(self._n_dec):
            p = f"decoder.block.{i}.layer"
            attn(p + ".0.SelfAttention", i == 0)
            _register(self, p + ".0.layer_norm.weight", P(d))
            attn(p + ".1.EncDecAttention", False)
            _register(self, p + ".1.layer_norm.weight", P(d))
            ff(p + ".2")
            _register(self, p + ".2.layer_norm.weight", P(d))
        _register(self, "decoder.final_layer_norm.weight", P(d))
        if self.use_position_embedding:
            pos = P(self.max_item_num + 1, d)
            _register(self, "position_embedding.weight", pos)
            _register(self, "encoder.position_embedding.weight", pos)
        _register(self, "lm_head.weight", shared if getattr(c, "tie_word_embeddings", True) else P(V, d))
        self._init_weights()
        self._packed = None
        self._version = 0
        self._workspace = None
        self._tries: Dict[int, tuple] = {}
        self._precision = os.environ.get("GRAM_PRECISION") or None
        if self._precision is not None and self._precision not in self.PRECISIONS:
            raise ValueError(f"GRAM_PRECISION={self._precision!r}: choose from {self.PRECISIONS}")
        self._pcache = None
        self._stage_caps: Dict[str, int] = {}

    def _init_weights(self) -> None:
        c = self.config
        d, dk, H, F = c.d_model, c.d_kv, c.num_heads, c.d_ff
        with torch.no_grad():
            for name, p in self.named_parameters():
                if name.endswith("layer_norm.weight"):
                    p.fill_(1.0)
                elif name.endswith(".q.weight"):
                    p.normal_(0.0, (d * dk) ** -0.5)
                elif name.endswith((".k.weight", ".v.weight", "wi.weight", "relative_attention_bias.weight")):
                    p.normal_(0.0, d ** -0.5)
                elif name.endswith(".o.weight"):
                    p.normal_(0.0, (H * dk) ** -0.5)
                elif name.endswith("wo.weight"):
                    p.normal_(0.0, F ** -0.5)
                elif name.endswith("position_embedding.weight"):
                    p.normal_(0.0, 0.02)
                else:
                    p.normal_(0.0, 1.0)

    def load_state_dict(self, state_dict, strict: bool = True, **kw):
        out = super().load_state_dict(state_dict, strict=strict, **kw)
        self._invalidate()
        return out

    def load_t5(self, state_dict):
        remapped = {}
        for k, v in state_dict.items():
            if k.startswith("encoder.block."):
                parts = k.split(".")
                k = "encoder.encoder.block." + parts[2] + ".module." + ".".join(parts[3:])
            elif k.startswith("encoder.") and not k.startswith("encoder.encoder."):
                k = "encoder." + k
            remapped[k] = v
        return self.load_state_dict(remapped, strict=False)

    PRECISIONS = ("bf16", "bf16x3", "f16", "f16x3")
    _PIECES = {"bf16": 1, "bf16x3": 2, "f16": 1, "f16x3": 2}

    @staticmethod
    def default_precision() -> str:
        return "f16x3" if _lib.load().gram_piece_format() == 1 else "bf16x3"

    @property
    def precision(self) -> str:
        if self._precision is None:
# ... 459 lines not shown
            dec_wqkv=ptr_array([qkv(dd.format(i) + ".0.SelfAttention", dd.format(i) + ".0.layer_norm.weight", "dec_self") for i in range(nd)]),
            dec_wo=ptr_array([b16(sd[dd.format(i) + ".0.SelfAttention.o.weight"], "dec_self") for i in range(nd)]),
            dec_ln2=ptr_array([f32(sd[dd.format(i) + ".1.layer_norm.weight"]) for i in range(nd)]),
            dec_wq_x=ptr_array([lin(dd.format(i) + ".1.EncDecAttention.q.weight", dd.format(i) + ".1.layer_norm.weight", "dec_cross") for i in range(nd)]),
            dec_wo_x=ptr_array([b16(sd[dd.format(i) + ".1.EncDecAttention.o.weight"], "dec_cross") for i in range(nd)]),
            dec_ln3=ptr_array([f32(sd[dd.format(i) + ".2.layer_norm.weight"]) for i in range(nd)]),
            dec_wi=ptr_array([lin(dd.format(i) + ".2.DenseReluDense.wi.weight", dd.format(i) + ".2.layer_norm.weight", "dec_ffn") for i in range(nd)]),
            dec_wo2=ptr_array([b16(sd[dd.format(i) + ".2.DenseReluDense.wo.weight"], "dec_ffn") for i in range(nd)]),
            dec_wkv_x_all=b16(wkv_all, None, kv_row_caps),
            pieces=pieces, lm_head_f32=f32(sd["lm_head.weight"]) if pieces > 1 else None,
        )
        assert len(w_scales) == 4 * ne + 6 * nd + 2
        order = w_scales[1:] + w_scales[:1]
        arr = (C.c_float * len(order))(*order)
        keep.append(arr)
        desc.w_scales = C.cast(arr, C.POINTER(C.c_float))
        handle = lib.gram_model_create(C.byref(desc))
        if not handle:
            raise _lib.GramHipError("gram_model_create rejected the configuration (dims must be multiples of 128, heads <= 16)")
        self._packed = (dev, self._version, handle, keep)
        if self._max_passage_len != _lib.GRAM_MAX_PASSAGE_LEN:
            _lib.check(lib.gram_model_set_max_passage_len(handle, self._max_passage_len), "gram_model_set_max_passage_len")
        if self._max_fused_tokens != _lib.GRAM_MAX_FUSED_LEN:
            _lib.check(lib.gram_model_set_max_fused_len(handle, self._max_fused_tokens), "gram_model_set_max_fused_len")
        self._build_token_tables(handle, keep)
        return handle

    def _build_token_tables(self, handle, keep) -> None:
        lib = _lib.load()
        self._token_tables = None
        need = lib.gram_token_tables_bytes(handle)
        if need <= 0 or os.environ.get("GRAM_TOKEN_TABLES", "1") == "0":
            return
        dev = self._device()
        tables = torch.empty(int(need), dtype=torch.uint8, device=dev)
        scratch = torch.empty(int(lib.gram_token_tables_workspace_bytes(handle)), dtype=torch.uint8, device=dev)
        with torch.cuda.device(dev):
            _lib.check(lib.gram_model_build_token_tables(handle, tables.data_ptr(), tables.numel(), scratch.data_ptr(), scratch.numel(),
                                                         torch.cuda.current_stream(dev).cuda_stream), "gram_model_build_token_tables")
        keep.append(tables)
        self._token_tables = tables

    def _get_workspace(self, handle, B, N, L, K, max_length) -> torch.Tensor:
        lib = _lib.load()
        need = lib.gram_workspace_bytes(handle, B, N, L, K, max_length)
        if need < 0:
            raise _lib.GramHipError(
                f"unsupported problem size B={B} N={N} L={L} K={K} max_length={max_length} "
                f"(N <= max_item_num+1, L <= {self._max_passage_len}, N*L <= {self._max_fused_tokens}, K <= 64, max_length <= {_lib.GRAM_MAX_DEC_LEN}; "
                f"the Trie's fan-out is not limited)"
            )
        return self._ensure_workspace(need)

    def _ensure_workspace(self, need: int) -> torch.Tensor:
        dev = self._device()
        if self._workspace is None or self._workspace.device != dev or self._workspace.numel() < need:
            self._workspace = None
            torch.cuda.empty_cache()
            self._workspace = torch.empty(int(need), dtype=torch.uint8, device=dev)
        return self._workspace

    def max_users_per_call(self, N: int, L: int, K: int, max_length: int, limit: int = 4096, headroom: float = 0.9) -> int:
        self._check_fused_len(N, L)
        handle = self._pack()
        lib = _lib.load()
        dev = self._device()
        Lp = (int(L) + 31) // 32 * 32
        torch.cuda.empty_cache()
        free, _total = torch.cuda.mem_get_info(dev)
        if self._workspace is not None and self._workspace.device == dev:
            free += self._workspace.numel()
        budget = int(free * headroom)
        lo, hi = 1, max(1, int(limit))
        if lib.gram_workspace_bytes(handle, hi, N, Lp, K, max_length) <= budget:
            return hi
        while lo < hi:
            mid = (lo + hi + 1) // 2
            need = lib.gram_workspace_bytes(handle, mid, N, Lp, K, max_length)
            if 0 <= need <= budget:
                lo = mid
            else:
                hi = mid - 1
        return lo

    @staticmethod
    def _closure_trie(fn: Callable):
        for cell in getattr(fn, "__closure__", None) or ():
            obj = cell.cell_contents
            if isinstance(obj, Trie):
                return obj
            if hasattr(obj, "trie_dict") and hasattr(obj, "get"):
                return obj
        return None

    def _flat_trie(self, fn: Callable) -> FlatTrie:
        trie = self._closure_trie(fn)
        cached = self._tries.get(id(trie))
        if cached is None or cached[0] is not trie or cached[1].n_sequences != len(trie):
            cached = (trie, FlatTrie(trie))
            self._tries = {id(trie): cached}
        return cached[1]

    _CACHE_L = _lib.GRAM_MAX_PASSAGE_LEN
    _KEY_MULT: Dict[tuple, torch.Tensor] = {}

    @staticmethod
    def _canonical(rows_ids: torch.Tensor, rows_mask: torch.Tensor, width: int = _lib.GRAM_MAX_PASSAGE_LEN) -> torch.Tensor:
        canon = torch.where(rows_mask.bool(), rows_ids, rows_ids.new_full((), -1)).to(torch.int32)
        if canon.shape[1] > width:
            raise ValueError(f"passages of {canon.shape[1]} tokens do not fit the passage cache's rows of {width}")
        return torch.nn.functional.pad(canon, (0, width - canon.shape[1]), value=-1)

    @staticmethod
    def _passage_keys(canon: torch.Tensor) -> torch.Tensor:
        width = int(canon.shape[1])
        mult = GRAM._KEY_MULT.get((canon.device, width))
        if mult is None:
            g = torch.Generator().manual_seed(0x6772616D)
            mult = torch.randint(1, 2 ** 31 - 1, (width,), generator=g, dtype=torch.int64).to(canon.device)
            GRAM._KEY_MULT[(canon.device, width)] = mult
        return ((canon.to(torch.int64) + 1) * mult).sum(dim=1)

    def _pcache_rows(self, n_new: int):
        dev, d = self._device(), self.config.d_model
        pc = self._pcache
        used = 0 if pc is None else pc["n"]
        cap = 0 if pc is None else pc["x"].shape[0]
        if used + n_new > cap:
            new_cap = max(used + n_new, 2 * cap, int(getattr(self, "_pcache_reserve", 0)))
            x = torch.empty(new_cap, self._CACHE_L, d, dtype=torch.float32, device=dev)
            canon = torch.full((new_cap, self._CACHE_L), -1, dtype=torch.int32, device=dev)
# ... 132 lines not shown
    @torch.no_grad()
    def generate(self, input_ids, attention_mask, max_length, prefix_allowed_tokens_fn=None, num_beams=1,
                 num_return_sequences=None, output_scores=True, return_dict_in_generate=True, length_penalty=1.0,
                 exclude_items=None, allowed_items=None, candidates=None, **unused):
        if prefix_allowed_tokens_fn is None:
            raise NotImplementedError("unconstrained generation is not on GRAM's scoring path (a Trie is always passed)")
        neutral = {"do_sample": False, "early_stopping": False, "num_beam_groups": 1, "repetition_penalty": 1.0,
                   "no_repeat_ngram_size": 0, "diversity_penalty": 0.0, "use_cache": True, "temperature": 1.0, "top_k": 50,
                   "top_p": 1.0, "min_length": 0, "pad_token_id": 0, "eos_token_id": 1, "decoder_start_token_id": 0}
        for k, v in unused.items():
            if k in neutral:
                if v is not None and v != neutral[k] and k not in ("temperature", "top_k", "top_p"):
                    raise NotImplementedError(f"generate({k}={v!r}) is not supported by the HIP scoring path "
                                              f"(only {k}={neutral[k]!r}, the value the GRAM runners use)")
            elif v is not None:
                import warnings
                warnings.warn(f"gram_amd.GRAM.generate ignores the keyword argument {k!r}")
        if input_ids.dim() != 3:
            raise ValueError("input_ids must be (B, N, L)")
        self._check_passage_len(input_ids.shape[-1])
        self._check_fused_len(input_ids.shape[1], input_ids.shape[2])
        handle = self._pack()
        lib = _lib.load()
        dev = self._device()
        K = int(num_beams)
        nret = int(num_return_sequences or K)
        B, N, L = input_ids.shape
        ids = input_ids.to(dev, torch.int64)
        mask = attention_mask.to(dev).ne(0).view(torch.uint8) if attention_mask.dtype != torch.bool else attention_mask.to(dev).view(torch.uint8)
        Lp = (L + 31) // 32 * 32
        if Lp != L:
            ids = torch.nn.functional.pad(ids, (0, Lp - L))
            mask = torch.nn.functional.pad(mask, (0, Lp - L))
        ids, mask = ids.contiguous(), mask.contiguous()
        filtered = exclude_items is not None or allowed_items is not None
        if exclude_items is not None and allowed_items is not None:
            raise ValueError("generate: exclude_items and allowed_items are mutually exclusive")
        if filtered and candidates is None:
            raise ValueError("generate: exclude_items / allowed_items index `candidates` (the sequences the Trie was built from): pass it")
        if filtered and self._closure_trie(prefix_allowed_tokens_fn) is None:
            raise ValueError("generate: exclude_items / allowed_items need the Trie closure form of prefix_allowed_tokens_fn "
                             "(an arbitrary callback receives batch_id and can filter per user itself)")
        if self._closure_trie(prefix_allowed_tokens_fn) is None:
            if K == 1:
                raise NotImplementedError("greedy search needs the Trie closure form of prefix_allowed_tokens_fn")
            return self._generate_with_callback(ids, mask, B, N, Lp, K, nret, int(max_length), float(length_penalty),
                                                prefix_allowed_tokens_fn, return_dict_in_generate)
        flat = self._flat_trie(prefix_allowed_tokens_fn)
        if filtered:
            allow = allowed_items is not None
            items = self._user_item_lists(allowed_items if allow else exclude_items, allow, B, flat, candidates, dev)
        comp, harvest_plan = self._plan(ids, mask, B, N, Lp)
        _ctrie, (t_off, t_tok, t_node) = flat.to_device(dev)
        ws = self._get_workspace(handle, B, N, Lp, K, int(max_length))
        if K == 1 and nret != 1:
            raise ValueError("num_return_sequences must be 1 for greedy search (num_beams == 1), as in HF generate")
        ct = comp[2] if comp else dict(comp_map=None, comp_ids=None, comp_mask=None, cache_slot=None, cache_x=None, n_cached=0, cache_L=0)
        from .. import ops as _ops
        args = (ids, mask, int(handle), ws, t_off, t_tok, t_node, int(flat.max_fanout), int(flat.min_seq_len), K, nret, int(max_length),
                float(length_penalty), ct["comp_map"], ct["comp_ids"], ct["comp_mask"], ct["cache_slot"], ct["cache_x"],
                int(ct["n_cached"]), int(ct["cache_L"]))
        if filtered:
            leaf_lo, leaf_hi = flat.leaf_ranges_on(dev)
            seqs, scores, width = torch.ops.gram.generate_items(*args, leaf_lo, leaf_hi, flat.item_ranks_on(dev, candidates)[1], items,
                                                                allow)
        else:
            seqs, scores, width = torch.ops.gram.generate(*args)
        if harvest_plan is not None:
            self._harvest_from_workspace(harvest_plan, ws, handle, B, N, Lp, K, int(max_length))
        seqs = seqs[:, : int(width[0])]
        scores = scores if K > 1 else None
        if not return_dict_in_generate:
            return seqs
        return GenerateOutput(sequences=seqs, sequences_scores=scores)

    @staticmethod
    def _user_item_lists(lists, allow: bool, B: int, flat: FlatTrie, candidates, device="cpu") -> torch.Tensor:
        what = "allowed_items" if allow else "exclude_items"
        limit = _lib.GRAM_MAX_USER_ITEMS
        if isinstance(lists, torch.Tensor):
            if lists.dim() != 2 or lists.shape[0] != B or lists.dtype.is_floating_point or lists.dtype == torch.bool:
                raise ValueError(f"generate: {what} must be a (B, M) integer tensor padded with -1, or B lists")
            t = lists.detach().to(device, torch.int64)
        else:
            rows = [list(map(int, r)) for r in lists]
            if len(rows) != B:
                raise ValueError(f"generate: {what} needs one list per user ({B}), got {len(rows)}")
            t = torch.full((B, max(1, max(map(len, rows)))), -1, dtype=torch.int64)
            for b, r in enumerate(rows):
                t[b, : len(r)] = torch.tensor(r, dtype=torch.int64)
            t = t.to(device)
        if t.shape[1] == 0:
            t = torch.full((B, 1), -1, dtype=torch.int64, device=device)
        n = len(candidates)
        if n < 1:
            raise ValueError(f"generate: {what} indexes an empty `candidates`")
        valid = t != -1
        outside = (t < -1) | (t >= n)
        per_user = valid.sum(dim=1)
        t = torch.gather(t, 1, torch.sort((~valid).to(torch.uint8), dim=1, stable=True).indices)
        if torch.device(device).type == "cpu":
            rank = torch.from_numpy(flat.item_ranks(candidates))
        else:
            rank = flat.item_ranks_on(device, candidates)[1]
        r = torch.where((t >= 0) & (t < n), rank.to(torch.int64)[t.clamp(0, n - 1)], torch.full_like(t, -1)).sort(dim=1).values
        distinct = (r[:, :1] >= 0).sum(dim=1) + ((r[:, 1:] != r[:, :-1]) & (r[:, 1:] >= 0)).sum(dim=1)
        empty = distinct == 0 if allow else distinct >= int(flat.leaf_ranges()[1][0])
        any_outside, longest, any_empty, first_empty = torch.stack(
            [outside.any().long(), per_user.max(), empty.any().long(), empty.long().argmax()]).tolist()
        if any_outside:
            raise ValueError(f"generate: {what} holds an index outside [0, {n}) (-1 is the padding value)")
        if longest > limit:
            raise ValueError(f"generate: {what} has {longest} entries for one user, at most {limit} are supported")
        if any_empty:
            raise ValueError(f"generate: {what} leaves user {first_empty} without any item")
        return t[:, : max(1, longest)].to(torch.int32).contiguous()

    @torch.no_grad()
    def sequence_items(self, sequences, prefix_allowed_tokens_fn, candidates):
        flat = self._flat_trie(prefix_allowed_tokens_fn)
# ... 78 lines not shown
```

### gram_amd/ops.py

```python
from __future__ import annotations

import ctypes as C
from typing import List, Optional, Tuple

import torch

from . import _lib

Tensor = torch.Tensor


def _stream(t: Tensor) -> int:
    return torch.cuda.current_stream(t.device).cuda_stream


def _p(t: Optional[Tensor]):
    return None if t is None else t.data_ptr()


def _check(name: str, t: Tensor, dtype, shape=None, device=None, contiguous: bool = True) -> None:
    if t.dtype != dtype:
        raise ValueError(f"{name}: dtype {t.dtype}, expected {dtype}")
    if device is not None and t.device != device:
        raise ValueError(f"{name}: on {t.device}, expected {device}")
    if contiguous and not t.is_contiguous():
        raise ValueError(f"{name}: must be contiguous (got strides {t.stride()})")
    if t.numel() and t.data_ptr() % 16:
        raise ValueError(f"{name}: data pointer must be 16-byte aligned")
    if shape is not None:
        if t.dim() != len(shape) or any(e is not None and int(s_) != int(e) for s_, e in zip(t.shape, shape)):
            raise ValueError(f"{name}: shape {tuple(t.shape)}, expected {tuple('*' if e is None else e for e in shape)}")


@torch.library.custom_op("gram::generate", mutates_args=("workspace",), device_types="cuda")
def generate(input_ids: Tensor, attention_mask: Tensor, handle: int, workspace: Tensor, trie_child_off: Tensor,
             trie_child_tok: Tensor, trie_child_node: Tensor, trie_max_fanout: int, trie_min_seq_len: int, num_beams: int,
             num_return_sequences: int, max_length: int, length_penalty: float, comp_map: Optional[Tensor],
             comp_ids: Optional[Tensor], comp_mask: Optional[Tensor], cache_slot: Optional[Tensor], cache_x: Optional[Tensor],
             n_cached: int, cache_L: int) -> Tuple[Tensor, Tensor, Tensor]:
    lib = _lib.load()
    B, N, L = input_ids.shape
    dev = input_ids.device
    K, nret = num_beams, num_return_sequences
    trie = _lib.Trie(trie_child_off.data_ptr(), trie_child_tok.data_ptr(), trie_child_node.data_ptr(), trie_child_off.numel() - 1,
                     trie_child_tok.numel(), trie_max_fanout, trie_min_seq_len)
    comp = None
    if comp_map is not None:
        comp = _lib.Compaction(comp_map.numel(), comp_map.data_ptr(), _p(comp_ids), _p(comp_mask), n_cached, cache_L, _p(cache_x),
                               _p(cache_slot))
    seqs = torch.empty(B * nret, max_length, dtype=torch.int64, device=dev)
    scores = torch.empty(B * nret if K > 1 else 0, dtype=torch.float32, device=dev)
    width = C.c_int32(0)
    with torch.cuda.device(dev):
        rc = lib.gram_generate_ex(handle, input_ids.data_ptr(), attention_mask.data_ptr(), B, N, L, K, nret, max_length,
                                  float(length_penalty), C.byref(trie), C.byref(comp) if comp is not None else None,
                                  workspace.data_ptr(), workspace.numel(), seqs.data_ptr(), scores.data_ptr() if K > 1 else None,
                                  C.byref(width), _stream(input_ids))
    _lib.check(rc, "gram_generate")
    return seqs, scores, torch.tensor([width.value], dtype=torch.int32)


@generate.register_fake
def _(input_ids, attention_mask, handle, workspace, trie_child_off, trie_child_tok, trie_child_node, trie_max_fanout,
      trie_min_seq_len, num_beams, num_return_sequences, max_length, length_penalty, comp_map, comp_ids, comp_mask, cache_slot,
      cache_x, n_cached, cache_L):
    B = input_ids.shape[0]
    return (input_ids.new_empty(B * num_return_sequences, max_length),
            input_ids.new_empty(B * num_return_sequences if num_beams > 1 else 0, dtype=torch.float32),
            torch.empty(1, dtype=torch.int32))


@torch.library.custom_op("gram::generate_items", mutates_args=("workspace",), device_types="cuda")
def generate_items(input_ids: Tensor, attention_mask: Tensor, handle: int, workspace: Tensor, trie_child_off: Tensor,
                   trie_child_tok: Tensor, trie_child_node: Tensor, trie_max_fanout: int, trie_min_seq_len: int, num_beams: int,
                   num_return_sequences: int, max_length: int, length_penalty: float, comp_map: Optional[Tensor],
                   comp_ids: Optional[Tensor], comp_mask: Optional[Tensor], cache_slot: Optional[Tensor], cache_x: Optional[Tensor],
                   n_cached: int, cache_L: int, leaf_lo: Tensor, leaf_hi: Tensor, item_rank: Tensor, items: Tensor,
                   allow: bool) -> Tuple[Tensor, Tensor, Tensor]:
    lib = _lib.load()
    if input_ids.dim() != 3 or items.dim() != 2:
        raise ValueError("generate_items: input_ids must be (B, N, L) and items (B, M)")
    B, N, L = input_ids.shape
    dev = input_ids.device
    K, nret = num_beams, num_return_sequences
    M = items.shape[1]
    n_nodes = trie_child_off.numel() - 1
    _check("input_ids", input_ids, torch.int64)
    _check("attention_mask", attention_mask, torch.uint8, (B, N, L), dev)
    for name, t, shape in (("trie_child_off", trie_child_off, None), ("trie_child_tok", trie_child_tok, None),
                           ("trie_child_node", trie_child_node, (trie_child_tok.numel(),)), ("leaf_lo", leaf_lo, (n_nodes,)),
                           ("leaf_hi", leaf_hi, (n_nodes,)), ("item_rank", item_rank, (None,)), ("items", items, (B, None))):
        _check(name, t, torch.int32, shape, dev)
    if n_nodes < 1 or item_rank.numel() < 1 or not 1 <= M <= _lib.GRAM_MAX_USER_ITEMS:
        raise ValueError(f"generate_items: need a Trie, at least one candidate and 1 <= M <= {_lib.GRAM_MAX_USER_ITEMS} (got M={M})")
    lo_i, hi_i = torch.stack([items.min(), items.max()]).tolist()
    if lo_i < -1 or hi_i >= item_rank.numel():
        raise ValueError(f"generate_items: items must lie in [0, {item_rank.numel()}) or be the padding value -1")
    trie = _lib.Trie(trie_child_off.data_ptr(), trie_child_tok.data_ptr(), trie_child_node.data_ptr(), n_nodes,
                     trie_child_tok.numel(), trie_max_fanout, trie_min_seq_len)
    comp = None
    if comp_map is not None:
        comp = _lib.Compaction(comp_map.numel(), comp_map.data_ptr(), _p(comp_ids), _p(comp_mask), n_cached, cache_L, _p(cache_x),
                               _p(cache_slot))
    ranks = torch.empty(B, M, dtype=torch.int32, device=dev)
    count = torch.empty(B, dtype=torch.int32, device=dev)
    ui = _lib.UserItems(leaf_lo.data_ptr(), leaf_hi.data_ptr(), ranks.data_ptr(), count.data_ptr(), M,
                        _lib.ITEMS_ALLOW if allow else _lib.ITEMS_EXCLUDE)
    seqs = torch.empty(B * nret, max_length, dtype=torch.int64, device=dev)
    scores = torch.empty(B * nret if K > 1 else 0, dtype=torch.float32, device=dev)
    width = C.c_int32(0)
    with torch.cuda.device(dev):
        _lib.check(lib.gram_user_items_prepare(item_rank.data_ptr(), item_rank.numel(), items.data_ptr(), B, M, ranks.data_ptr(),
                                               count.data_ptr(), M, _stream(input_ids)), "gram_user_items_prepare")
        rc = lib.gram_generate_items(handle, input_ids.data_ptr(), attention_mask.data_ptr(), B, N, L, K, nret, max_length,
                                     float(length_penalty), C.byref(trie), C.byref(comp) if comp is not None else None, C.byref(ui),
                                     workspace.data_ptr(), workspace.numel(), seqs.data_ptr(), scores.data_ptr() if K > 1 else None,
                                     C.byref(width), _stream(input_ids))
    _lib.check(rc, "gram_generate_items")
# ... 353 lines not shown
```

### gram_amd/runner/base.py

```python
from __future__ import annotations

import logging
import os
from time import time
from typing import List, Optional, Sequence

import numpy as np
import torch

from ..utils import evaluate
from ..utils import generation_trie as gt

SPLIT_TOKENS = (1820, 9175)


def _arg(args, name, default):
    return getattr(args, name, default) if args is not None else default


class _PredRows:

    def __init__(self, gold, items, scores, extra, cand_str, K):
        self.gold, self.items, self.scores, self.extra, self.cand_str, self.K = gold, items, scores, extra, cand_str, K

# ... 69 lines not shown
        if _arg(self.args, "datasets", None) and _arg(self.args, "data_path", None):
            small = bool(_arg(self.args, "debug_test_small_set", False))
            (self.get_testloader if mode == "test" else self.get_validloader)(regenerate=False, phase=0, debug_test_small_set=small)
        loaders = self.testloaders if mode == "test" else self.validloaders
        if not loaders:
            raise RuntimeError(f"no {mode} loader: pass args.datasets/args.data_path (the reference's flags) or fill "
                               f"runner.{'testloaders' if mode == 'test' else 'validloaders'} before calling")
        return loaders

    def encode_candidates(self, candidates: Sequence) -> List[List[int]]:
        if len(candidates) and not isinstance(candidates[0], str):
            return [list(map(int, c)) for c in candidates]
        id_type = _arg(self.args, "item_id_type", "split")
        out = []
        for cand in candidates:
            if id_type == "t5_token":
                out.append([0] + self.tokenizer.convert_tokens_to_ids(cand.split(" ")) + [1])
            elif id_type == "split":
                out.append([0] + [t for t in self.tokenizer.encode(cand) if t not in SPLIT_TOKENS])
            else:
                out.append([0] + self.tokenizer.encode(f"{cand}"))
        return out

    def _load(self, path: Optional[str], strict: bool = True) -> None:
        if path:
            if os.path.isdir(path):
                path = os.path.join(path, os.listdir(path)[0])
            self.model.load_state_dict(torch.load(path, map_location=self.device, weights_only=True), strict=strict)

    def _generate_model(self):
        return self.model_rec.module if hasattr(self.model_rec, "module") else self.model_rec

    def _warm_passage_cache(self, testloader, chunk: int = 2048) -> int:
        mode = int(_arg(self.args, "passage_cache", 1))
        model = self._generate_model()
        if hasattr(model, "set_passage_harvest"):
            model.set_passage_harvest(mode == 1)
        item2input = getattr(testloader.dataset, "item2input", None)
        if not mode or not item2input or not hasattr(model, "cache_passages"):
            return 0
        if hasattr(model, "reserve_passage_cache"):
            model.reserve_passage_cache(len(set(item2input.values())))
        encode = getattr(getattr(testloader, "collate_fn", None), "encode_passages", None)
        if mode != 2 or encode is None:
            return 0
        texts = sorted(set(item2input.values()))
        start, n = time(), 0
        for lo in range(0, len(texts), chunk):
            ids, mask = encode(texts[lo:lo + chunk])
            n = model.cache_passages(ids, mask)
        logging.info(f"passage cache: {n} item prompts encoded in {time() - start:.2f}s")
        return n

    def _gpu_batch_users(self, model, n_slots: int, L: int, K: int, max_length: int) -> int:
        explicit = int(_arg(self.args, "eval_gpu_batch", 0) or os.environ.get("GRAM_EVAL_USERS", 0) or 0)
        if explicit > 0:
            return explicit
        if hasattr(model, "max_users_per_call"):
            return int(model.max_users_per_call(n_slots, L, K, max_length, limit=4096))
        return 4096

    def _rescore_unfinished(self, model, input_ids, attention_mask, seqs, scores, fn, K, ref_max_length, shape):
        B = input_ids.shape[0]
        unfinished = (~torch.isfinite(scores.view(B, K))).any(dim=1).nonzero().flatten()
        if unfinished.numel() == 0:
            return seqs, scores
        per_call = int(model.max_users_per_call(shape[0], shape[1], K, ref_max_length, limit=4096)) if hasattr(model, "max_users_per_call") \
            else int(unfinished.numel())
        width = seqs.shape[1]
        redo = []
        for lo in range(0, int(unfinished.numel()), max(per_call, 1)):
            u = unfinished[lo:lo + per_call]
            redo.append(model.generate(input_ids=input_ids[u], attention_mask=attention_mask[u], max_length=ref_max_length,
                                       prefix_allowed_tokens_fn=fn, num_beams=K, num_return_sequences=K, output_scores=True,
                                       return_dict_in_generate=True, length_penalty=self.length_penalty))
            width = max(width, redo[-1]["sequences"].shape[1])
        out_seqs = seqs.new_zeros(B * K, width)
        out_seqs[:, : seqs.shape[1]] = seqs
        out_scores = scores.clone()
        rows_of = lambda u: (u[:, None] * K + torch.arange(K, device=u.device)[None, :]).flatten()
        lo = 0
        for r in redo:
            n = r["sequences"].shape[0] // K
            rows = rows_of(unfinished[lo:lo + n].to(out_seqs.device))
            out_seqs[rows] = 0
            out_seqs[rows, : r["sequences"].shape[1]] = r["sequences"].to(out_seqs.device)
            out_scores[rows.to(out_scores.device)] = r["sequences_scores"].to(out_scores.device)
            lo += n
        return out_seqs, out_scores

    @staticmethod
    def _merge_batches(parts):
        if len(parts) == 1:
            return parts[0]
        B = sum(p["item_text_ids"].shape[0] for p in parts)
        N = max(p["item_text_ids"].shape[1] for p in parts)
        L = max(p["item_text_ids"].shape[2] for p in parts)
        T = max(p["target_ids"].shape[1] for p in parts)
        ids = torch.zeros(B, N, L, dtype=parts[0]["item_text_ids"].dtype)
        mask = torch.zeros(B, N, L, dtype=torch.bool)
        tgt = torch.full((B, T), -100, dtype=parts[0]["target_ids"].dtype)
        users, lo = [], 0
        for p in parts:
            b, n, l = p["item_text_ids"].shape
            ids[lo:lo + b, :n, :l] = p["item_text_ids"]
            mask[lo:lo + b, :n, :l] = p["item_text_masks"].bool()
            tgt[lo:lo + b, : p["target_ids"].shape[1]] = p["target_ids"]
            users += list(p.get("user_ids", [None] * b))
            lo += b
        return {"item_text_ids": ids, "item_text_masks": mask, "target_ids": tgt, "user_ids": users}

    def _gpu_batches(self, testloader, users_per_call: int):
# ... 39 lines not shown
        if prompt_len > 128 and hasattr(gen_model, "set_max_passage_len") and getattr(gen_model, "_max_passage_len", 128) != prompt_len:
            gen_model.set_max_passage_len(prompt_len)
        fused = (int(_arg(self.args, "max_his", 20)) + 1) * prompt_len
        if fused > 4096 and hasattr(gen_model, "set_max_fused_tokens"):
            fused = min(16384, (fused + 31) // 32 * 32)
            if getattr(gen_model, "_max_fused_tokens", 4096) != fused:
                gen_model.set_max_fused_tokens(fused)

    def _score_loader(self, testloader):
        import queue
        import threading

        phases = {}
        t_phase = time()

        def lap(name):
            nonlocal t_phase
            now = time()
            phases[name] = phases.get(name, 0.0) + now - t_phase
            t_phase = now

        self._raise_model_limits(testloader)
        self._warm_passage_cache(testloader)
        lap("passage_cache")
        candidates = testloader.dataset.all_items
        encoded = self.encode_candidates(candidates)
        trie = gt.Trie(encoded)
        fn = gt.prefix_allowed_tokens_fn(trie)
        lap("candidates_and_trie")
        longest = max(len(c) for c in encoded)
        ref_max_length = longest
        if isinstance(candidates[0], str) and _arg(self.args, "item_id_type", "split") not in ("t5_token", "split"):
            ref_max_length = 50
        max_length = min(longest, ref_max_length)
        K = self.generate_num
        model = self._generate_model()
        on_device_items = hasattr(model, "sequence_items")
        cand_str = self._decode_rows(encoded)
        str2sid = {}
        for i, s in enumerate(cand_str):
            str2sid.setdefault(s, i)
        cand_sid = np.fromiter((str2sid[s] for s in cand_str), dtype=np.int64, count=len(cand_str))
        other_sid = {}

        def sid_of(s):
            r = str2sid.get(s)
            if r is None:
                r = other_sid.setdefault(s, -2 - len(other_sid))
            return r

        collator = getattr(testloader, "collate_fn", None)
        n_slots = int(_arg(self.args, "max_his", 20)) + 1
        L = int(getattr(collator, "item_prompt_max_len", 0) or _arg(self.args, "item_prompt_max_len", 128))
        users_per_call = self._gpu_batch_users(model, n_slots, L, K, max_length)
        lap("candidate_strings")
        logging.info(f"scoring {users_per_call} users per generate() call (--eval_batch_size {_arg(self.args, 'eval_batch_size', 1)} "
                     f"is the loader's; results do not depend on the batch)")

        batches_q: "queue.Queue" = queue.Queue(maxsize=2)
        post_q: "queue.Queue" = queue.Queue(maxsize=4)
        failure = []

        def produce():
            try:
                for batch in self._gpu_batches(testloader, users_per_call):
                    batches_q.put(batch)
            except BaseException as e:
                failure.append(e)
            batches_q.put(None)

        out = dict(ranks=[], user_ids=[], gold=[], items=[], scores=[], extra=[])

        def post_one(batch, items, scores, seqs):
            B = scores.shape[0]
            gold = self._decode(batch["target_ids"])
            gold_sid = np.fromiter((sid_of(g) for g in gold), dtype=np.int64, count=B)
            extra = {}
            if items is None:
                gen = self._decode(seqs)
                pred_sid = np.fromiter((sid_of(s) for s in gen), dtype=np.int64, count=B * K).reshape(B, K)
                extra = dict(enumerate(gen))
                items = np.full((B, K), -1, dtype=np.int32)
            else:
                pred_sid = np.where(items >= 0, cand_sid[np.maximum(items, 0)], -1)
                miss = np.argwhere(items < 0)
                if len(miss):
                    strs = self._decode(seqs[miss[:, 0] * K + miss[:, 1]])
                    for (b, k), s in zip(miss.tolist(), strs):
                        pred_sid[b, k] = sid_of(s)
                        extra[b * K + k] = s
            out["ranks"].append(evaluate.hit_ranks_from_ids(pred_sid, scores, gold_sid))
            out["user_ids"] += list(batch.get("user_ids", [None] * B))
            out["gold"] += gold
            out["items"].append(items)
            out["scores"].append(scores)
            out["extra"].append(extra)

        def post():
            while True:
                job = post_q.get()
                if job is None:
                    return
                if failure:
                    continue
                try:
                    post_one(*job)
                except BaseException as e:
# ... 104 lines not shown
```

### gram_amd/utils/generation_trie.py

```python
from __future__ import annotations

from typing import Dict, Iterable, Iterator, List, Optional, Sequence

import numpy as np


class Trie:

    def __init__(self, sequences: Optional[Iterable[Sequence[int]]] = None):
        self._dict: Dict[int, dict] = {}
        self._pending: List[List[int]] = []
        self._sequences: Optional[List[List[int]]] = []
        self.len = 0
        self.append_trie = None
        self.bos_token_id = None
        for seq in sequences or ():
            self.add(seq)

    @property
    def trie_dict(self) -> Dict[int, dict]:
        if self._pending:
            pending, self._pending = self._pending, []
            for seq in pending:
                node = self._dict
# ... 251 lines not shown

        n = self.n_nodes
        fan = np.diff(self.child_off).astype(np.int64)
        root_toks = self.child_tok[int(self.child_off[0]):int(self.child_off[1])]
        if int(start_token) not in root_toks.tolist():
            raise ValueError(f"decoder_rows: no candidate starts with the decoder start token {int(start_token)}")
        if len(root_toks) != 1:
            raise ValueError(f"decoder_rows: a candidate starts with a token other than the decoder start token {int(start_token)} "
                             f"(generate could never return it: its score is undefined)")
        child = self.child_node.astype(np.int64)
        parent = np.zeros(n, dtype=np.int64)
        parent[child] = np.repeat(np.arange(n, dtype=np.int64), fan)
        node_tok = np.full(n, -1, dtype=np.int64)
        node_tok[child] = self.child_tok
        depth = np.zeros(n, dtype=np.int64)
        levels, frontier = [], np.zeros(1, dtype=np.int64)
        while frontier.size:
            levels.append(frontier)
            counts = fan[frontier]
            first = self.child_off[frontier].astype(np.int64)
            edges = np.repeat(first - (np.cumsum(counts) - counts), counts) + np.arange(int(counts.sum()), dtype=np.int64)
            frontier = child[edges]
            depth[frontier] = len(levels)
        internal = (fan > 0) & (np.arange(n) > 0)
        row_node = np.nonzero(internal)[0]
        Q = int(row_node.size)
        if Q < 1:
            raise ValueError("decoder_rows: the Trie has no candidate longer than the start token")
        row_of = np.full(n, -1, dtype=np.int64)
        row_of[row_node] = np.arange(Q)
        pos = depth[row_node] - 1
        Tq = int(pos.max()) + 1
        if Tq > _lib.GRAM_MAX_DEC_LEN:
            raise ValueError(f"decoder_rows: the longest candidate needs {Tq} decoder positions; at most {_lib.GRAM_MAX_DEC_LEN} "
                             f"(GRAM_MAX_DEC_LEN) are supported")
        if (np.diff(pos) < 0).any():
            raise ValueError("decoder_rows: the Trie's nodes are not numbered level by level")
        anc = np.zeros((Q, Tq), dtype=np.int64)
        parent_row = row_of[parent[row_node]]
        for t in range(Tq):
            rows = np.nonzero(pos == t)[0]
            if t:
                anc[rows, :t] = anc[parent_row[rows], :t]
            anc[rows, t] = rows
        lo, hi = self.leaf_ranges()
        leaf = (fan == 0) & (np.arange(n) > 0)
        out = DecoderRows(tokens=node_tok[row_node].astype(np.int32), pos=pos.astype(np.int32), anc=anc.astype(np.int32),
                          row_node=row_node.astype(np.int32), node_row=row_of[parent].astype(np.int32), node_tok=node_tok.astype(np.int32),
                          node_leaf=np.where(leaf, lo, -1).astype(np.int32), Q=Q, Tq=Tq, n_nodes=n, n_leaves=int(hi[0]))
        out.node_row[0] = -1
        self._decoder_rows[int(start_token)] = out
        return out

    def decoder_rows_on(self, device, start_token: int = 0):
        import torch

        key = ("rows", str(device), int(start_token))
        if key not in self._device:
            rows = self.decoder_rows(start_token)
            self._device[key] = (rows, tuple(torch.from_numpy(np.ascontiguousarray(getattr(rows, f))).to(device) for f in DecoderRows.ARRAYS))
        return self._device[key]

    def item_ranks(self, candidates: Sequence[Sequence[int]]) -> np.ndarray:
        n = len(candidates)
        if n == 0:
            return np.zeros(0, dtype=np.int32)
        lens = np.fromiter((len(c) for c in candidates), dtype=np.int64, count=n)
        width = int(lens.max())
        toks = np.full((n, max(width, 1)), -1, dtype=np.int64)
        for i, c in enumerate(candidates):
            toks[i, : len(c)] = c
        node = np.zeros(n, dtype=np.int64)
        fan = np.diff(self.child_off)
        edge_key = np.repeat(np.arange(self.n_nodes, dtype=np.int64), fan) * (1 << 32) + self.child_tok.astype(np.int64)
        for p in range(width):
            live = (lens > p) & (node >= 0)
            if not live.any() or not len(edge_key):
                node[live] = -1
                continue
            key = node[live] * (1 << 32) + toks[live, p]
            e = np.minimum(np.searchsorted(edge_key, key), len(edge_key) - 1)
            node[live] = np.where(edge_key[e] == key, self.child_node[e], -1)
        if (node < 0).any():
            raise ValueError(f"item_ranks: candidate {int(np.nonzero(node < 0)[0][0])} is not in the Trie")
        bad = (fan[node] != 0) | (node == 0)
        if bad.any():
            raise ValueError(f"item_ranks: candidate {int(np.nonzero(bad)[0][0])} does not end on a leaf of the Trie")
        return self.leaf_ranges()[0][node].astype(np.int32)

    def get(self, prefix: Sequence[int]) -> List[int]:
        node = 0
        for tok in prefix:
            lo, hi = int(self.child_off[node]), int(self.child_off[node + 1])
            i = lo + int(np.searchsorted(self.child_tok[lo:hi], tok))
            if i >= hi or self.child_tok[i] != tok:
                return []
            node = int(self.child_node[i])
        return self.child_tok[self.child_off[node]:self.child_off[node + 1]].tolist()

    def to_device(self, device):
        import torch
        from .. import _lib

        key = str(device)
        if key not in self._device:
            t_off = torch.from_numpy(self.child_off).to(device)
# ... 39 lines not shown
```

### include/gram_hip.h

```cpp
#ifndef GRAM_HIP_H
#define GRAM_HIP_H

#include <stddef.h>
#include <stdint.h>

#ifdef __cplusplus
extern "C" {
#endif

#define GRAM_ABI_VERSION 7

#define GRAM_E_ARG (-1)
#define GRAM_E_WORKSPACE (-2)
#define GRAM_E_BEAM (-3)
#define GRAM_E_NONFINITE (-4)

#define GRAM_MAX_BEAMS 64
#define GRAM_MAX_DEC_LEN 64
#define GRAM_MAX_PASSAGE_LEN 128
#define GRAM_MAX_LONG_PASSAGE_LEN 512
#define GRAM_MAX_FUSED_LEN 4096
#define GRAM_MAX_LONG_FUSED_LEN 16384

enum gram_epilogue {
// ... 232 lines not shown
  const float* w_scales;
} gram_model_desc_t;

typedef struct gram_model gram_model_t;

gram_model_t* gram_model_create(const gram_model_desc_t* desc_host);
void gram_model_destroy(gram_model_t* m);

int gram_model_set_max_passage_len(gram_model_t* m, int Lmax);

int gram_model_set_max_fused_len(gram_model_t* m, int Smax);

int gram_iota_i32(int32_t* out, int n, void* stream);
int64_t gram_token_tables_bytes(const gram_model_t* m);
int64_t gram_token_tables_workspace_bytes(const gram_model_t* m);
int gram_model_build_token_tables(gram_model_t* m, void* tables, int64_t tables_bytes, void* workspace, int64_t workspace_bytes,
                                  void* stream);

int64_t gram_workspace_bytes(const gram_model_t* m, int B, int N, int L, int K, int max_length);

int gram_encode_fused(const gram_model_t* m, const int64_t* input_ids, const uint8_t* mask, int B, int N,
                      int L, void* workspace, int64_t workspace_bytes, int K, int max_length,
                      void* enc_out_bf16, void* stream);

int gram_decode_step(const gram_model_t* m, const int32_t* tokens, const int32_t* anc, const uint8_t* mask,
                     int B, int N, int L, int K, int max_length, int t, void* workspace,
                     int64_t workspace_bytes, float* logits, void* stream);

int gram_generate(const gram_model_t* m, const int64_t* input_ids, const uint8_t* mask, int B, int N, int L,
                  int K, int nret, int max_length, float length_penalty, const gram_trie_t* trie_host,
                  void* workspace, int64_t workspace_bytes, int64_t* sequences, float* scores,
                  int32_t* width_host, void* stream);

typedef struct {
  int32_t n_active;
  const int32_t* passage_map;
  const int64_t* ids;
  const uint8_t* mask;
  int32_t n_cached;
  int32_t cache_L;
  const float* cache_x;
  const int32_t* cache_slot;
} gram_compaction_t;
int gram_generate_ex(const gram_model_t* m, const int64_t* input_ids, const uint8_t* mask, int B, int N, int L,
                     int K, int nret, int max_length, float length_penalty, const gram_trie_t* trie_host,
                     const gram_compaction_t* compaction_host, void* workspace, int64_t workspace_bytes,
                     int64_t* sequences, float* scores, int32_t* width_host, void* stream);

int gram_generate_items(const gram_model_t* m, const int64_t* input_ids, const uint8_t* mask, int B, int N, int L, int K, int nret,
                        int max_length, float length_penalty, const gram_trie_t* trie_host, const gram_compaction_t* compaction_host,
                        const gram_user_items_t* items_host, void* workspace, int64_t workspace_bytes, int64_t* sequences,
                        float* scores, int32_t* width_host, void* stream);

int gram_encode_passages(const gram_model_t* m, const int64_t* ids, const uint8_t* mask, int P, int L,
                         void* workspace, int64_t workspace_bytes, float* x_out, void* stream);
int64_t gram_workspace_encoder_x_offset(const gram_model_t* m, int B, int N, int L, int K, int max_length);
int gram_gather_passage_x(const float* cache_x, const int32_t* slot, float* x, int n, int L, int cache_L, int d,
                          void* stream);


int64_t gram_workspace_bytes_tf(const gram_model_t* m, int B, int N, int L, int C, int T);

int gram_teacher_forced(const gram_model_t* m, const int64_t* input_ids, const uint8_t* mask, int B, int N, int L,
                        const gram_compaction_t* compaction_host, const int32_t* dec_ids, const int32_t* labels, int C, int T,
                        void* workspace, int64_t workspace_bytes, float* logits, float* token_logp, float* seq_logp, void* stream);

int gram_dec_self_attn_tf_split(const void* qkv, const float* bias, void* out, int n_seq, int T, int H, int pieces,
                                int64_t qkv_pstride, void* stream);

int gram_cross_attn_rows_split(const void* q, const void* k_layer, const void* vt_layer, const uint8_t* mask, void* out, int B, int Q,
                               int H, int S, int pieces, int64_t q_pstride, int64_t bank_pstride, const uint32_t* key_bits,
                               int32_t* rowmap, void* stream);
int gram_cross_attn_rows_long_split(const void* q, const void* k_layer, const void* vt_layer, const uint8_t* mask, void* out, int B,
                                    int Q, int H, int S, int pieces, int64_t q_pstride, int64_t bank_pstride, const uint32_t* key_bits,
                                    float* scratch, int32_t* rowmap, void* stream);

int gram_label_logprob_split(const void* hidden, const void* lm_head_bf16, const float* lm_head_f32, int d, const float* lse,
                             const int32_t* labels, int n_seq, int T, int V, int pieces, float* token_logp, float* seq_logp,
                             void* stream);


int gram_cross_attn_probs_split(const void* q, const void* k_layer, const uint8_t* mask, float* probs, int B, int Q, int H, int S,
                                int pieces, int64_t q_pstride, int64_t bank_pstride, const uint32_t* key_bits, void* stream);

int gram_xattn_head_sum(const float* probs, float* acc, int B, int Q, int H, int S, int first, void* stream);

int gram_xattn_passage_scores(const float* acc, const uint8_t* mask, float* scores, int B, int Q, int N, int L, float denom,
                              void* stream);

typedef struct {
  float* probs;
  float* layer_probs;
  float* token_scores;
  float* passage_scores;
} gram_xattn_out_t;

int gram_teacher_forced_ex(const gram_model_t* m, const int64_t* input_ids, const uint8_t* mask, int B, int N, int L,
                           const gram_compaction_t* compaction_host, const int32_t* dec_ids, const int32_t* labels, int C, int T,
                           void* workspace, int64_t workspace_bytes, float* logits, float* token_logp, float* seq_logp,
                           const gram_xattn_out_t* attn_host, void* stream);


typedef struct {
  const int32_t* tokens;
  const int32_t* pos;
  const int32_t* anc;
  const int32_t* row_node;
  const int32_t* node_row;
  const int32_t* node_tok;
  const int32_t* node_leaf;
  int32_t Q, Tq;
  int32_t n_nodes, n_leaves;
} gram_trie_rows_t;

int gram_dec_self_attn_tree_split(const void* qkv, const int32_t* pos, const int32_t* anc, const float* bias, void* out, int B, int Q,
                                  int Tq, int H, int pieces, int64_t qkv_pstride, void* stream);

int gram_trie_repeat_tokens(const int32_t* tokens, int32_t* out, int B, int Q, void* stream);

int gram_trie_leaf_logprob_split(const void* hidden, const void* lm_head_bf16, const float* lm_head_f32, int d, const float* lse,
                                 const gram_trie_rows_t* rows_host, int B, int V, int pieces, float* row_edge, float* leaf_logp,
                                 float* node_logp, void* stream);

int64_t gram_workspace_bytes_trie(const gram_model_t* m, int B, int N, int L, int Q);

int gram_score_trie(const gram_model_t* m, const int64_t* input_ids, const uint8_t* mask, int B, int N, int L,
                    const gram_compaction_t* compaction_host, const gram_trie_t* trie_host, const gram_trie_rows_t* rows_host,
                    void* workspace, int64_t workspace_bytes, float* leaf_logp, float* node_logp, void* stream);

enum gram_kernel_kind {
  GRAM_K_GEMM = 0,
  GRAM_K_ENC_ATTN = 1,
  GRAM_K_CROSS_ATTN = 2,
  GRAM_K_DEC_SELF_ATTN = 3,
  GRAM_K_ROWOPS = 4,
  GRAM_K_LSE = 5,
  GRAM_K_BEAM = 6,
  GRAM_K_COUNT = 7
};
int gram_prof_enable(uint32_t kind_mask, int max_events);
int gram_prof_reset(void);
int gram_prof_collect(int kind, double* total_ms, int64_t* launches, double* work, int64_t* dropped);

int gram_prof_pp_clock_enable(int on);
int gram_prof_pp_clock(double* ghz, int reset);

int gram_debug_set_gemm_variant(int variant);

int gram_debug_stream_read(const void* src, size_t bytes, void* sink, void* stream);
int gram_debug_stream_read_variant(const void* src, size_t bytes, void* sink, int variant, int wgs, void* stream);

int gram_debug_set_live_rows(int on);
int gram_debug_set_token_tables(int on);
int gram_debug_set_beam_chunked(int mode);
int gram_debug_set_beam_chunk_capacity(int candidates);
enum gram_stage {
  GRAM_STAGE_ENC_ATTN = 0,
  GRAM_STAGE_ENC_FFN = 1,
  GRAM_STAGE_BANK_K = 2,
  GRAM_STAGE_BANK_V = 3,
  GRAM_STAGE_DEC_SELF = 4,
  GRAM_STAGE_DEC_CROSS = 5,
  GRAM_STAGE_DEC_FFN = 6,
  GRAM_STAGE_LM_HEAD = 7,
  GRAM_STAGE_COUNT = 8
};
int gram_debug_set_stage_pieces(const int32_t* caps, int n);

int gram_gemm_f16(const void* A, const void* W, void* C, int M, int N, int K, int lda, int ldc, int epilogue,
                  const gram_kv_bank_t* bank_host, void* stream);
int gram_gemm_f16_ex(const void* A, const void* W, void* C, int M, int N, int K, int lda, int ldc, int epilogue,
                     const gram_kv_bank_t* bank_host, const gram_norm_fusion_t* nf_host, void* stream);
int gram_gemm_f16_split(const void* A, const void* W, void* C, int M, int N, int kc, int lda, int ldc, int epilogue,
                        const gram_kv_bank_t* bank_host, const gram_norm_fusion_t* nf_host, const gram_split_t* split_host, void* stream);
int gram_gemm_f16_lse(const void* A, const void* W, float* logits, float* lse_part, int M, int N, int K, int lda, int ldc, void* stream);
int gram_gemm_f16_lse_split(const void* A, const void* W, float* logits, float* lse_part, int M, int N, int kc, int lda, int ldc,
                            const gram_split_t* split_host, void* stream);
int gram_rmsnorm_f16(const float* x, const float* w, void* out_f16, int rows, int d, float eps, float scale, const float* pos, int N,
                     int L, void* stream);
int gram_rmsnorm_f16_map(const float* x, const float* w, void* out_f16, int rows, int d, float eps, float scale, const float* pos,
                         int N, int L, const int32_t* passage_map, void* stream);
int gram_rmsnorm_f16_split(const float* x, const float* w, void* out_f16, int rows, int d, float eps, float scale, const float* pos,
                           int N, int L, const int32_t* passage_map, int pieces, void* stream);

int gram_abi_version(void);
int gram_piece_format(void);

#ifdef __cplusplus
}
#endif
#endif
```

Before: 3119.

## Decode trie tail in one forest pass instead of per-step beam decoding

Adds a tail-forest generation path. When every remaining node in the constrained trie below a depth threshold expands into a bounded subtree, all live beams' remaining subtrees are expanded into a flat forest of rows. Those rows are decoded level by level, using grouped cross-attention entries, row scatter and ancestor tables, in place of many sequential beam steps. The aim is to cut per-step launch and beam-search overhead in the last decode steps. The cost is extra workspace, new trie preprocessing on the host, and a more complex scheduling path with capacity fallbacks.

```diff
diff --git a/gram_amd/_lib.py b/gram_amd/_lib.py
--- a/gram_amd/_lib.py
+++ b/gram_amd/_lib.py
@@ -17,6 +17,8 @@
 K_GEMM, K_ENC_ATTN, K_CROSS_ATTN, K_DEC_SELF_ATTN, K_ROWOPS, K_LSE, K_BEAM = range(7)
 E_ARG, E_WORKSPACE, E_BEAM, E_NONFINITE = -1, -2, -3, -4
 ABI_VERSION = 7
+GRAM_TAIL_ENTRY_ROWS = 64
+GRAM_TAIL_MAX_STEPS = 16
 GRAM_MAX_USER_ITEMS = 4096
 ITEMS_EXCLUDE, ITEMS_ALLOW = 0, 1
 MAX_PIECES = 2
@@ -88,6 +90,16 @@
 class TrieRows(C.Structure):
     _fields_ = [("tokens", vp), ("pos", vp), ("anc", vp), ("row_node", vp), ("node_row", vp), ("node_tok", vp), ("node_leaf", vp),
                 ("Q", i32), ("Tq", i32), ("n_nodes", i32), ("n_leaves", i32)]
+
+
+class TrieTail(C.Structure):
+    _fields_ = [("sub_rows", vp), ("d_tail", i32), ("steps", i32)]
+
+
+class Forest(C.Structure):
+    _fields_ = [("tokens", vp), ("pos", vp), ("parent", vp), ("root", vp), ("node", vp), ("user_off", vp), ("ent_off", vp),
+                ("ent_users", vp), ("ent_rows", vp), ("rowpos", vp), ("counts", vp), ("slot", vp), ("lvl_rows", vp), ("lvl_tokens", vp),
+                ("lvl_anc", vp), ("cap_rows", i32), ("cap_entries", i32), ("n_levels", i32), ("pad_", i32)]
 
 
 class ModelDesc(C.Structure):
@@ -214,6 +226,20 @@
     "gram_workspace_bytes_trie": (i64, [vp, C.c_int, C.c_int, C.c_int, C.c_int]),
     "gram_score_trie": (C.c_int, [vp, vp, vp, C.c_int, C.c_int, C.c_int, C.POINTER(Compaction), C.POINTER(Trie), C.POINTER(TrieRows), vp,
                                   i64, vp, vp, vp]),
+    "gram_tail_forest": (C.c_int, [C.POINTER(BeamState), C.POINTER(Trie), C.POINTER(TrieTail), C.POINTER(Forest), C.c_int, vp]),
+    "gram_tail_rowpos": (C.c_int, [C.POINTER(BeamState), C.POINTER(Trie), C.POINTER(Forest), vp]),
+    "gram_scatter_rows": (C.c_int, [vp, vp, vp, C.c_int, C.c_int, C.c_int, vp]),
+    "gram_cross_attn_entries_split": (C.c_int, [vp, vp, vp, vp, vp, C.c_int, C.c_int, C.c_int, C.c_int, vp, vp, C.c_int, i64, i64, vp,
+                                                vp]),
+    "gram_workspace_bytes_tail": (i64, [vp, C.c_int, C.c_int, C.c_int, C.c_int, C.c_int, C.c_int]),
+    "gram_generate_tail": (C.c_int, [vp, vp, vp, C.c_int, C.c_int, C.c_int, C.c_int, C.c_int, C.c_int, f32, C.POINTER(Trie),
+                                     C.POINTER(Compaction), C.POINTER(TrieTail), vp, i64, vp, vp, C.POINTER(i32), vp]),
+    "gram_debug_set_tail_pass": (C.c_int, [C.c_int]),
+    "gram_tail_pass_wanted": (C.c_int, [vp, C.c_int, C.c_int, C.c_int]),
+    "gram_debug_set_tail_capacity": (C.c_int, [C.c_int]),
+    "gram_debug_set_tail_level_capacity": (C.c_int, [C.c_int]),
+    "gram_debug_tail_last": (C.c_int, [C.POINTER(i32)]),
+    "gram_debug_workspace_beam_state": (C.c_int, [vp, vp, C.c_int, C.c_int, C.c_int, C.c_int, C.c_int, C.POINTER(BeamState)]),
 }
 
 for _old, _new in (("gram_gemm_bf16", "gram_gemm_f16"), ("gram_gemm_bf16_ex", "gram_gemm_f16_ex"), ("gram_gemm_bf16_split", "gram_gemm_f16_split"),
diff --git a/gram_amd/csrc/beam.hip b/gram_amd/csrc/beam.hip
--- a/gram_amd/csrc/beam.hip
+++ b/gram_amd/csrc/beam.hip
@@ -974,6 +974,188 @@
   out_item[r] = item;
 }
 
+__device__ __forceinline__ bool tail_live(const gram_beam_state_t& st, const gram_trie_t& tr, int b, int row) {
+  if (st.done[b]) return false;
+  const int nd = st.node[row];
+  return nd >= 0 && nd < tr.n_nodes && tr.child_off[nd + 1] > tr.child_off[nd];
+}
+
+__global__ __launch_bounds__(1024) void tail_count_kernel(gram_beam_state_t st, gram_trie_t tr, gram_trie_tail_t tl, gram_forest_t f) {
+  __shared__ long long s_w[16], s_tot;
+  __shared__ int s_mx[16];
+  const int tid = threadIdx.x, lane = tid & 63, wave = tid >> 6;
+  const int K = st.K, B = st.B;
+  auto scan = [&](long long v) {
+    for (int o = 1; o < 64; o <<= 1) {
+      const long long n = __shfl_up(v, o, 64);
+      if (lane >= o) v += n;
+    }
+    gram_sync();
+    if (lane == 63) s_w[wave] = v;
+    gram_sync();
+    if (tid == 0) {
+      long long acc = 0;
+      for (int w = 0; w < 16; ++w) {
+        const long long t = s_w[w];
+        s_w[w] = acc;
+        acc += t;
+      }
+      s_tot = acc;
+    }
+    gram_sync();
+    return v + s_w[wave];
+  };
+  const long long sat = (long long)f.cap_rows + 1;
+  long long rbase = 0, ebase = 0;
+  int mx = 0;
+  for (int c0 = 0; c0 < B; c0 += 1024) {
+    const int b = c0 + tid;
+    long long n = 0;
+    if (b < B) {
+      for (int k = 0; k < K; ++k)
+        if (tail_live(st, tr, b, b * K + k)) {
+          const int s = tl.sub_rows[st.node[b * K + k]];
+          n += s > 0 ? s : 0;
+        }
+      n = n > sat ? sat : n;
+    }
+    const long long e = (n + GRAM_TAIL_ENTRY_ROWS - 1) / GRAM_TAIL_ENTRY_ROWS;
+    const long long ri = scan(n);
+    const long long r0 = rbase + ri - n;
+    rbase += s_tot;
+    const long long ei = scan(e);
+    const long long e0 = ebase + ei - e;
+    ebase += s_tot;
+    if (b < B) {
+      f.user_off[b] = (int)(r0 > INT32_MAX ? INT32_MAX : r0);
+      f.ent_off[b] = (int)(e0 > INT32_MAX ? INT32_MAX : e0);
+      mx = n > mx ? (int)n : mx;
+    }
+  }
+  mx = (int)wave_max((float)mx);
+  if (lane == 0) s_mx[wave] = mx;
+  gram_sync();
+  if (tid == 0) {
+    for (int w = 1; w < 16; ++w) mx = s_mx[w] > mx ? s_mx[w] : mx;
+    f.user_off[B] = (int)(rbase > INT32_MAX ? INT32_MAX : rbase);
+    f.ent_off[B] = (int)(ebase > INT32_MAX ? INT32_MAX : ebase);
+    f.counts[0] = f.user_off[B];
+    f.counts[1] = f.ent_off[B];
+    f.counts[2] = mx;
+    f.counts[3] = 0;
+    for (int l = 0; l < 2 * GRAM_TAIL_MAX_STEPS; ++l) f.counts[4 + l] = 0;
+  }
+}
+
+__global__ __launch_bounds__(64) void tail_fill_kernel(gram_beam_state_t st, gram_trie_t tr, gram_forest_t f, int t) {
+  const int b = blockIdx.x * 64 + threadIdx.x;
+  if (b >= st.B) return;
+  if (f.counts[0] > f.cap_rows || f.counts[1] > f.cap_entries) return;
+  const int K = st.K, base = f.user_off[b], cnt = f.user_off[b + 1] - base;
+  auto put = [&](int i, int tok, int pos, int parent, int root, int node) {
+    f.tokens[i] = tok;
+    f.pos[i] = pos;
+    f.parent[i] = parent;
+    f.root[i] = root;
+    f.node[i] = node;
+  };
+  int n = 0;
+  for (int k = 0; k < K && n < cnt; ++k)
+    if (tail_live(st, tr, b, b * K + k)) {
+      put(base + n, st.tokens[b * K + k], t, -1, b * K + k, st.node[b * K + k]);
+      ++n;
+    }
+  for (int head = 0; head < n && n < cnt; ++head) {
+    const int row = base + head, nd = f.node[row];
+    const int e1 = tr.child_off[nd + 1];
+    for (int e = tr.child_off[nd]; e < e1 && n < cnt; ++e) {
+      const int c = tr.child_node[e];
+      if (c >= 0 && c < tr.n_nodes && tr.child_off[c + 1] > tr.child_off[c]) {
+        put(base + n, tr.child_tok[e], f.pos[row] + 1, row, f.root[row], c);
+        ++n;
+      }
+    }
+  }
+  if (n < cnt) {
+    st.error[0] = 3;
+    for (; n < cnt; ++n) put(base + n, st.pad, t, -1, b * K, -1);
+  }
+  const int grp = b & 1;
+  for (int i = 0; i < cnt;) {
+    const int l = f.pos[base + i] - t;
+    int j = i + 1;
+    while (j < cnt && f.pos[base + j] - t == l) ++j;
+    const bool ok = l >= 0 && l < f.n_levels;
+    const int s0 = ok ? atomicAdd(&f.counts[4 + grp * GRAM_TAIL_MAX_STEPS + l], j - i) : 0;
+    const size_t tab = ((size_t)grp * f.n_levels + (ok ? l : 0)) * f.cap_rows;
+    for (int k = i; k < j; ++k) {
+      const int sl = s0 + (k - i);
+      f.slot[base + k] = ok && sl < f.cap_rows ? sl : -1;
+      if (ok && sl < f.cap_rows) {
+        f.lvl_rows[tab + sl] = base + k;
+        f.lvl_tokens[tab + sl] = f.tokens[base + k];
+      }
+    }
+    i = j;
+  }
+  const int e0 = f.ent_off[b], ne = f.ent_off[b + 1] - e0;
+  for (int e = 0; e < ne; ++e) {
+    f.ent_users[e0 + e] = b;
+    for (int s = 0; s < GRAM_TAIL_ENTRY_ROWS; ++s) {
+      const int i = e * GRAM_TAIL_ENTRY_ROWS + s;
+      f.ent_rows[(size_t)(e0 + e) * GRAM_TAIL_ENTRY_ROWS + s] = i < cnt ? base + i : -1;
+    }
+  }
+}
+
+__global__ __launch_bounds__(256) void tail_anc_kernel(gram_beam_state_t st, gram_forest_t f, int t) {
+  const int i = blockIdx.x * 256 + threadIdx.x;
+  const int n = f.counts[0], R = st.B * st.K;
+  if (n > f.cap_rows || f.counts[1] > f.cap_entries || i >= n) return;
+  const int l = f.pos[i] - t, s = f.slot[i];
+  if (l < 0 || l >= f.n_levels || s < 0 || s >= R) return;
+  int root = f.root[i];
+  root = root < 0 ? 0 : (root >= R ? R - 1 : root);
+  const int grp = (root / st.K) & 1;
+  int32_t* tab = f.lvl_anc + ((size_t)grp * f.n_levels + l) * st.Tmax * R;
+  for (int j = 0; j < t; ++j) tab[(size_t)j * R + s] = st.anc[(size_t)j * R + root];
+  int a = f.parent[i];
+  for (int u = 0; u < GRAM_TAIL_MAX_STEPS && a >= 0 && a < n; ++u) {
+    const int pa = f.pos[a], sa = f.slot[a];
+    if (pa >= t && pa < st.Tmax && sa >= 0 && sa < R) tab[(size_t)pa * R + s] = sa;
+    a = f.parent[a];
+  }
+}
+
+__global__ __launch_bounds__(256) void scatter_rows_kernel(const uint4* __restrict__ src, const int32_t* __restrict__ rows,
+                                                           uint4* __restrict__ dst, int n, int row16, int dst_rows) {
+  const long g = (long)blockIdx.x * 256 + threadIdx.x;
+  if (g >= (long)n * row16) return;
+  const int r = (int)(g / row16), c = (int)(g % row16);
+  const int d = rows[r];
+  if (d >= 0 && d < dst_rows) dst[(size_t)d * row16 + c] = src[g];
+}
+
+__global__ __launch_bounds__(256) void tail_rowpos_kernel(gram_beam_state_t st, gram_trie_t tr, gram_forest_t f) {
+  const int r = blockIdx.x * 256 + threadIdx.x;
+  if (r >= st.B * st.K) return;
+  const int b = r / st.K;
+  int pos = -1;
+  if (tail_live(st, tr, b, r)) {
+    const int nd = st.node[r], i1 = f.user_off[b + 1];
+    for (int i = f.user_off[b]; i < i1; ++i)
+      if (f.node[i] == nd) {
+        pos = i;
+        break;
+      }
+    if (pos < 0) {
+      st.error[0] = 3;
+      pos = 0;
+    }
+  }
+  f.rowpos[r] = pos;
+}
+
 }
 
 static int check_state(const gram_beam_state_t* st) {
@@ -1187,6 +1369,48 @@
   return 0;
 }
 
+static bool forest_ok(const gram_forest_t* f) {
+  return f && f->tokens && f->pos && f->parent && f->root && f->node && f->user_off && f->ent_off && f->ent_users && f->ent_rows &&
+         f->rowpos && f->counts && f->slot && f->lvl_rows && f->lvl_tokens && f->lvl_anc && f->cap_rows >= 1 && f->cap_entries >= 1 &&
+         f->n_levels >= 1 && f->n_levels <= GRAM_TAIL_MAX_STEPS;
+}
+
+extern "C" int gram_tail_forest(const gram_beam_state_t* st, const gram_trie_t* tr, const gram_trie_tail_t* tail,
+                                const gram_forest_t* forest, int t, void* stream) {
+  if (int e = check_state(st)) return e;
+  if (!tr || !tail || !tail->sub_rows || !forest_ok(forest) || t < 0 || t >= st->Tmax) return GRAM_E_ARG;
+  gram_prof::Scope prof(GRAM_K_BEAM, (hipStream_t)stream, 0.0);
+  hipLaunchKernelGGL(tail_count_kernel, dim3(1), dim3(1024), 0, (hipStream_t)stream, *st, *tr, *tail, *forest);
+  GRAM_CHECK_LAUNCH();
+  hipLaunchKernelGGL(tail_fill_kernel, dim3((st->B + 63) / 64), dim3(64), 0, (hipStream_t)stream, *st, *tr, *forest, t);
+  GRAM_CHECK_LAUNCH();
+  hipLaunchKernelGGL(tail_anc_kernel, dim3((forest->cap_rows + 255) / 256), dim3(256), 0, (hipStream_t)stream, *st, *forest, t);
+  GRAM_CHECK_LAUNCH();
+  return 0;
+}
+
+extern "C" int gram_scatter_rows(const void* src, const int32_t* rows, void* dst, int n, int row_bytes, int dst_rows, void* stream) {
+  if (!src || !rows || !dst || n < 1 || row_bytes < 16 || (row_bytes & 15) || dst_rows < 1 ||
+      ((reinterpret_cast<uintptr_t>(src) | reinterpret_cast<uintptr_t>(dst)) & 15))
+    return GRAM_E_ARG;
+  const int row16 = row_bytes / 16;
+  const long total = (long)n * row16;
+  gram_prof::Scope prof(GRAM_K_ROWOPS, (hipStream_t)stream, 2.0 * n * row_bytes);
+  hipLaunchKernelGGL(scatter_rows_kernel, dim3((unsigned)((total + 255) / 256)), dim3(256), 0, (hipStream_t)stream, (const uint4*)src, rows,
+                     (uint4*)dst, n, row16, dst_rows);
+  GRAM_CHECK_LAUNCH();
+  return 0;
+}
+
+extern "C" int gram_tail_rowpos(const gram_beam_state_t* st, const gram_trie_t* tr, const gram_forest_t* forest, void* stream) {
+  if (int e = check_state(st)) return e;
+  if (!tr || !forest_ok(forest)) return GRAM_E_ARG;
+  gram_prof::Scope prof(GRAM_K_BEAM, (hipStream_t)stream, 0.0);
+  hipLaunchKernelGGL(tail_rowpos_kernel, dim3((st->B * st->K + 255) / 256), dim3(256), 0, (hipStream_t)stream, *st, *tr, *forest);
+  GRAM_CHECK_LAUNCH();
+  return 0;
+}
+
 extern "C" int gram_greedy_step(const gram_beam_state_t* st, const gram_trie_t* tr, const float* logits, int V, int cur_len,
                                void* stream) {
   if (int e = check_state(st)) return e;
diff --git a/gram_amd/csrc/dec_attn.hip b/gram_amd/csrc/dec_attn.hip
--- a/gram_amd/csrc/dec_attn.hip
+++ b/gram_amd/csrc/dec_attn.hip
@@ -19,7 +19,7 @@
   return r;
 }
 
-template <int NT, bool LIVE, int S, int NW>
+template <int NT, bool LIVE, int S, int NW, bool ENT = false>
 __global__ __launch_bounds__(NW * 64) void cross_attn_kernel(
     const p16* __restrict__ q, const p16* __restrict__ kbank, const p16* __restrict__ vtbank,
     const uint8_t* __restrict__ mask, p16* __restrict__ out, int K, int H, int Sk, const int32_t* __restrict__ users,
@@ -35,6 +35,7 @@
   float* sm_o = sm_l + NW * NB;
 
   const int h = blockIdx.x, b = LIVE ? users[blockIdx.y] : blockIdx.y;
+  const int rb = ENT ? (int)blockIdx.y : b;
   const int tid = threadIdx.x, lane = tid & 63;
   const int wave = __builtin_amdgcn_readfirstlane(tid >> 6);
   const int c = lane & 15, g = lane >> 4;
@@ -56,7 +57,7 @@
 
 #pragma unroll
   for (int nt = 0; nt < NT; ++nt) {
-    const int qrow = xa_row<LIVE>(b, K, 16 * nt + c, rowpos);
+    const int qrow = xa_row<LIVE>(rb, K, 16 * nt + c, rowpos);
 #pragma unroll
     for (int pc = 0; pc < S; ++pc)
 #pragma unroll
@@ -249,7 +250,7 @@
       lt += __shfl_xor(lt, 16, 64);
       lt += __shfl_xor(lt, 32, 64);
       const float inv = 1.f / lt;
-      const int orow = xa_row<LIVE>(b, K, 16 * nt + c, rowpos);
+      const int orow = xa_row<LIVE>(rb, K, 16 * nt + c, rowpos);
       if (orow >= 0) {
 #pragma unroll
         for (int mt = 0; mt < 4; ++mt) xa_store<S>(out, orow, inner, h * 64 + 16 * mt + 4 * g, o[mt][nt] * inv);
@@ -279,7 +280,7 @@
     xa_merge_w(sm_m[beam], sm_m[NB + beam], sm_l[beam], sm_l[NB + beam], w0, w1, inv2);
     const f32x4 v = xa_merge_o(*reinterpret_cast<const f32x4*>(sm_o + ((size_t)beam) * 64 + d4),
                          *reinterpret_cast<const f32x4*>(sm_o + ((size_t)(NB + beam)) * 64 + d4), w0, w1, inv2);
-    int orow = b * K + beam;
+    int orow = rb * K + beam;
     if constexpr (LIVE) orow = rowpos[orow];
     if (orow >= 0) xa_store<S>(out, orow, inner, h * 64 + d4, v);
   }
@@ -333,6 +334,27 @@
   }
 }
 
+template <int S, int NW>
+int launch_cross_entries(const XaLaunch& a) {
+  constexpr int NT = 4, NB = NT * 16;
+  static_assert(NB == GRAM_TAIL_ENTRY_ROWS, "an entry's row table (gram_forest_t.ent_rows) is indexed by the kernel's padded row count");
+  constexpr int stages = NW * S * 2 * XA_TILE, merge = NW == 1 ? 0 : (2 * NW * NB + NW * NB * 64) * 4;
+  constexpr int smem = stages > merge ? stages : merge;
+  static_assert(smem <= 160 * 1024, "the stages do not fit the LDS");
+  static bool attr_set = false;
+  if (!attr_set) {
+    hipError_t e = hipFuncSetAttribute(reinterpret_cast<const void*>(cross_attn_kernel<NT, true, S, NW, true>),
+                                       hipFuncAttributeMaxDynamicSharedMemorySize, smem);
+    if (e != hipSuccess) return (int)e;
+    attr_set = true;
+  }
+  hipLaunchKernelGGL((cross_attn_kernel<NT, true, S, NW, true>), dim3(a.H, a.B), dim3(NW * 64), smem, a.st, (const p16*)a.q,
+                     (const p16*)a.k, (const p16*)a.vt, a.mask, (p16*)a.out, NB, a.H, a.Sk, a.users, a.rowpos, a.q_ps, a.bank_ps,
+                     a.key_bits);
+  GRAM_CHECK_LAUNCH();
+  return 0;
+}
+
 __global__ __launch_bounds__(128) void mask_key_bits_kernel(const uint8_t* __restrict__ mask, uint32_t* __restrict__ bits, int Sk) {
   const int b = blockIdx.x, st = threadIdx.x;
   uint32_t w = 0;
@@ -435,6 +457,25 @@
   }
 }
 
+}
+
+extern "C" int gram_cross_attn_entries_split(const void* q, const void* k_layer, const void* vt_layer, const uint8_t* mask, void* out,
+                                             int n_entries, int K, int H, int S, const int32_t* ent_users, const int32_t* ent_rows,
+                                             int pieces, int64_t q_pstride, int64_t bank_pstride, const uint32_t* key_bits,
+                                             void* stream) {
+  if (!q || !out || !ent_users || !ent_rows || n_entries < 1 || K < 1 || K > GRAM_MAX_BEAMS || H < 1 || S < 32 || (S & 31) ||
+      S > 4096 || pieces < 1 || pieces > GRAM_MAX_PIECES)
+    return GRAM_E_ARG;
+  if (pieces > 1 && (q_pstride < 1 || bank_pstride < (int64_t)H * S * 64)) return GRAM_E_ARG;
+  if ((reinterpret_cast<uintptr_t>(mask) & 15) || (reinterpret_cast<uintptr_t>(k_layer) & 15) || (reinterpret_cast<uintptr_t>(vt_layer) & 15))
+    return GRAM_E_ARG;
+  hipStream_t st = (hipStream_t)stream;
+  gram_prof::Scope prof(GRAM_K_CROSS_ATTN, st, 4.0 * n_entries * H * S * 64 * pieces);
+  const XaLaunch a{q, k_layer, vt_layer, mask, out, n_entries, GRAM_TAIL_ENTRY_ROWS, H, S, ent_users, ent_rows, (long)q_pstride,
+                   (long)bank_pstride, key_bits, st};
+  const bool one_wave = (K + 15) / 16 >= 3;
+  if (pieces == 2) return one_wave ? launch_cross_entries<2, 1>(a) : launch_cross_entries<2, 2>(a);
+  return one_wave ? launch_cross_entries<1, 1>(a) : launch_cross_entries<1, 2>(a);
 }
 
 extern "C" int gram_mask_key_bits(const uint8_t* mask, uint32_t* key_bits, int B, int S, void* stream) {
diff --git a/gram_amd/csrc/generate.hip b/gram_amd/csrc/generate.hip
--- a/gram_amd/csrc/generate.hip
+++ b/gram_amd/csrc/generate.hip
@@ -65,6 +65,10 @@
   float* xa_scratch;
   int32_t* rowmap;
   int64_t bytes;
+  gram_forest_t forest;
+  Rows tail;
+  float *tail_lse, *tail_lse_part;
+  int64_t tail_bytes;
   int pieces;
   int64_t ps_bank, ps_cache;
 };
@@ -149,6 +153,40 @@
   return w;
 }
 
+void carve_tail(const gram_model* m, void* ws, Workspace& w, int B, int K, int steps) {
+  const gram_model_desc_t& c = m->d;
+  const int64_t V = c.vocab, R = (int64_t)B * K;
+  Carve cv(ws);
+  cv.off = w.bytes;
+  const int64_t cap = (5 * R * steps + 3) / 4, ents = cap / GRAM_TAIL_ENTRY_ROWS + B;
+  gram_forest_t& f = w.forest;
+  f.cap_rows = (int32_t)cap;
+  f.cap_entries = (int32_t)ents;
+  f.tokens = cv.take<int32_t>(cap);
+  f.pos = cv.take<int32_t>(cap);
+  f.parent = cv.take<int32_t>(cap);
+  f.root = cv.take<int32_t>(cap);
+  f.node = cv.take<int32_t>(cap);
+  f.user_off = cv.take<int32_t>(B + 1);
+  f.ent_off = cv.take<int32_t>(B + 1);
+  f.ent_users = cv.take<int32_t>(ents);
+  f.ent_rows = cv.take<int32_t>(ents * GRAM_TAIL_ENTRY_ROWS);
+  f.rowpos = cv.take<int32_t>(R);
+  f.counts = cv.take<int32_t>(4 + 2 * GRAM_TAIL_MAX_STEPS);
+  f.n_levels = steps;
+  f.slot = cv.take<int32_t>(cap);
+  f.lvl_rows = cv.take<int32_t>(2 * cap * steps);
+  f.lvl_tokens = cv.take<int32_t>(2 * cap * steps);
+  f.lvl_anc = cv.take<int32_t>(2 * (int64_t)steps * GRAM_MAX_DEC_LEN * R);
+  w.tail = take_rows(cv, c, w.pieces, cap, true);
+  w.tail_lse = cv.take<float>(cap);
+  w.tail_lse_part = cv.take<float>(cap * (V / 64) * 2);
+  w.tail_bytes = (cv.off + 255) & ~(int64_t)255;
+}
+inline bool tail_shape_ok(int B, int K, int steps) {
+  return steps >= 1 && steps <= GRAM_TAIL_MAX_STEPS && 5 * (int64_t)B * K * steps / 4 + 1 <= INT32_MAX / 4;
+}
+
 int check_shapes(const gram_model* m, int B, int N, int L, int K, int Tmax) {
   if (!m || B < 1 || N < 1 || N > m->d.max_passages || L < 32 || L > m->max_L || (L & 31) || N * L > m->max_S || K < 1 ||
       K > GRAM_MAX_BEAMS || Tmax < 2 || Tmax > GRAM_MAX_DEC_LEN)
@@ -435,6 +473,101 @@
   return gram_beam_step_sparse(&w.beam, trie, w.dec.h, c.lm_head_bf16, c.d_model, w.lse, c.vocab, cur_len, rows_per_user, st);
 }
 
+int tail_pass(const gram_model* m, const Workspace& w, const uint8_t* mask, int B, int N, int L, int K, int Tmax, int t0, int n_rows,
+              int n_entries, const int32_t* lvl_n, void* st) {
+  const gram_model_desc_t& c = m->d;
+  const int inner = c.n_heads * 64, H = c.n_heads, S = N * L, R = B * K;
+  const size_t bank_layer = (size_t)B * H * S * 64;
+  const size_t cache_layer = (size_t)Tmax * R * inner;
+  const Rows& r = w.dec;
+  const gram_forest_t& f = w.forest;
+  const p16* const table = token_table(m, m->dec_qkv0, GRAM_STAGE_DEC_SELF);
+  int nlev = f.n_levels, cut = 0;
+  for (int g = 0; g < 2; ++g)
+    for (int l = 0; l < f.n_levels; ++l)
+      if (lvl_n[g * GRAM_TAIL_MAX_STEPS + l] > 0 && t0 + l >= Tmax - 1) cut = 1, nlev = l < nlev ? l : nlev;
+  TRY(decoder_layers(
+      m, w, f.tokens, n_rows, table != nullptr,
+      [&](int i) {
+        if (cut) {
+          hipError_t e = hipMemsetAsync(r.attn, 0, (size_t)n_rows * inner * w.pieces * sizeof(p16), (hipStream_t)st);
+          if (e != hipSuccess) return (int)e;
+        }
+        for (int g = 0; g < 2; ++g)
+          for (int l = 0; l < nlev; ++l) {
+            const int n = lvl_n[g * GRAM_TAIL_MAX_STEPS + l];
+            if (n < 1) continue;
+            const size_t tab = ((size_t)g * f.n_levels + l) * f.cap_rows;
+            const int32_t* const rows_l = f.lvl_rows + tab;
+            const int32_t* const anc_l = f.lvl_anc + ((size_t)g * f.n_levels + l) * Tmax * R;
+            if (i == 0 && table)
+              TRY(gram_dec_self_attn_rows_split(table, f.lvl_tokens + tab, w.kcache, w.vcache, anc_l, c.dec_bias_f32, r.qx, R, n, nullptr, H,
+                                                t0 + l, Tmax, w.pieces, (int64_t)c.vocab * 3 * inner, w.ps_cache, st));
+            else
+              TRY(gram_dec_self_attn_rows_split(r.qkv, rows_l, w.kcache + i * cache_layer, w.vcache + i * cache_layer, anc_l, c.dec_bias_f32,
+                                                r.qx, R, n, nullptr, H, t0 + l, Tmax, w.pieces, r.ps_qkv, w.ps_cache, st));
+            TRY(gram_scatter_rows(r.qx, rows_l, r.attn, n, inner * w.pieces * (int)sizeof(p16), n_rows, st));
+          }
+        return 0;
+      },
+      [&](int i) {
+        return gram_cross_attn_entries_split(r.qx, w.bank_k + i * bank_layer, w.bank_vt + i * bank_layer, mask, r.attn, n_entries, K, H, S,
+                                             f.ent_users, f.ent_rows, w.pieces, r.ps_qx, w.ps_bank, w.key_bits, st);
+      },
+      st));
+  TRY(lm_head(m, w, n_rows, nullptr, w.lse_part, st));
+  return gram_lse_combine(w.lse_part, w.lse, n_rows, c.vocab / 64, st);
+}
+Workspace tail_view(const Workspace& w) {
+  Workspace v = w;
+  v.dec = w.tail;
+  v.lse = w.tail_lse;
+  v.lse_part = w.tail_lse_part;
+  return v;
+}
+
+int g_tail_pass = -1;
+int g_tail_cap = 0;
+int g_tail_level_cap = 0;
+int32_t g_tail_last[4] = {0, 0, 0, 0};
+constexpr double kTailMinBankBytes = 256.0 * 1024 * 1024;
+bool tail_wanted(const gram_model* m, int B, int N, int L) {
+  if (g_tail_pass >= 0) return g_tail_pass != 0;
+  const char* e = getenv("GRAM_TAIL_PASS");
+  if (e && e[0] == '0') return false;
+  if (e && e[0] == '1') return true;
+  const int P = m->d.pieces > 1 ? m->d.pieces : 1;
+  return 4.0 * B * m->d.n_heads * N * L * 64 * P >= kTailMinBankBytes;
+}
+
+}
+
+extern "C" int gram_debug_set_tail_pass(int on) {
+  g_tail_pass = on;
+  return 0;
+}
+extern "C" int gram_tail_pass_wanted(const gram_model_t* m, int B, int N, int L) {
+  if (!m || B < 1 || N < 1 || L < 1) return GRAM_E_ARG;
+  return tail_wanted(m, B, N, L) ? 1 : 0;
+}
+extern "C" int gram_debug_set_tail_capacity(int rows) {
+  g_tail_cap = rows < 0 ? 0 : rows;
+  return 0;
+}
+extern "C" int gram_debug_workspace_beam_state(const gram_model_t* m, void* workspace, int B, int N, int L, int K, int max_length,
+                                               gram_beam_state_t* out) {
+  if (!workspace || !out || check_shapes(m, B, N, L, K, max_length)) return GRAM_E_ARG;
+  *out = carve(m, workspace, B, N, L, K, max_length).beam;
+  return 0;
+}
+extern "C" int gram_debug_set_tail_level_capacity(int rows) {
+  g_tail_level_cap = rows < 0 ? 0 : rows;
+  return 0;
+}
+extern "C" int gram_debug_tail_last(int32_t* out4) {
+  if (!out4) return GRAM_E_ARG;
+  memcpy(out4, g_tail_last, sizeof(g_tail_last));
+  return 0;
 }
 
 extern "C" int gram_abi_version(void) { return GRAM_ABI_VERSION; }
@@ -653,7 +786,7 @@
 namespace {
 int generate_body(const gram_model* m, Workspace& w, const int64_t* input_ids, const uint8_t* mask, int B, int N, int L, int K, int nret,
                   int max_length, const gram_trie_t* trie, const gram_compaction_t* comp, const gram_user_items_t* items,
-                  int64_t* sequences, float* scores, void* stream) {
+                  const gram_trie_tail_t* tail, int64_t* sequences, float* scores, void* stream) {
   TRY(encode_call(m, w, input_ids, mask, B, N, L, comp, stream));
   TRY(gram_beam_init(&w.beam, trie, 0, stream));
   if (K == 1) {
@@ -669,7 +802,36 @@
       return !(e && e[0] == '0');
     }();
     const bool live_rows = g_live_rows < 0 ? live_rows_env : g_live_rows != 0;
+    const int t_tail = tail ? tail->d_tail - 1 : -1;
+    bool replay = false;
+    Workspace wt = w;
+    if (tail) {
+      wt = tail_view(w);
+      if (g_tail_cap > 0 && g_tail_cap < wt.forest.cap_rows) wt.forest.cap_rows = g_tail_cap;
+    }
     for (int t = 0; t + 1 < max_length; ++t) {
+      if (t == t_tail) {
+        int32_t counts[4 + 2 * GRAM_TAIL_MAX_STEPS] = {0};
+        TRY(gram_tail_forest(&w.beam, trie, tail, &wt.forest, t, stream));
+        hipError_t e = hipMemcpyAsync(counts, wt.forest.counts, sizeof(counts), hipMemcpyDeviceToHost, (hipStream_t)stream);
+        if (e == hipSuccess) e = hipStreamSynchronize((hipStream_t)stream);
+        if (e != hipSuccess) return (int)e;
+        if (counts[0] < 0 || counts[1] < 0) return GRAM_E_BEAM;
+        g_tail_last[1] = counts[0], g_tail_last[2] = counts[1], g_tail_last[3] = counts[2];
+        bool fits = counts[0] >= 1 && counts[0] <= wt.forest.cap_rows && counts[1] >= 1 && counts[1] <= wt.forest.cap_entries;
+        const int level_cap = g_tail_level_cap > 0 && g_tail_level_cap < B * K ? g_tail_level_cap : B * K;
+        for (int l = 0; l < 2 * GRAM_TAIL_MAX_STEPS; ++l) fits = fits && counts[4 + l] >= 0 && counts[4 + l] <= level_cap;
+        if (fits) {
+          TRY(tail_pass(m, wt, mask, B, N, L, K, max_length, t, counts[0], counts[1], counts + 4, stream));
+          replay = true;
+          g_tail_last[0] = 1;
+        }
+      }
+      if (replay) {
+        TRY(gram_tail_rowpos(&w.beam, trie, &wt.forest, stream));
+        TRY(search_step(m, wt, trie, t + 1, K, wt.forest.rowpos, nullptr, stream));
+        continue;
+      }
       const int Kt = t == 0 ? 1 : K;
       if (live_rows && t >= 1 && trie->min_seq_len >= 2 && t >= trie->min_seq_len - 1) {
         int32_t counts[2] = {0, 0};
@@ -703,15 +865,26 @@
 
 static int generate_call(const gram_model_t* m, const int64_t* input_ids, const uint8_t* mask, int B, int N, int L, int K, int nret,
                          int max_length, float length_penalty, const gram_trie_t* trie, const gram_compaction_t* comp,
-                         const gram_user_items_t* items, void* workspace, int64_t workspace_bytes, int64_t* sequences, float* scores,
-                         int32_t* width_host, void* stream) {
+                         const gram_user_items_t* items, const gram_trie_tail_t* tail, void* workspace, int64_t workspace_bytes,
+                         int64_t* sequences, float* scores, int32_t* width_host, void* stream) {
   TRY(check_shapes(m, B, N, L, K, max_length));
   TRY(check_compaction(comp, B, N));
   if (!trie || nret < 1 || nret > K || !sequences || (!scores && K != 1)) return GRAM_E_ARG;
   Workspace w = carve(m, workspace, B, N, L, K, max_length);
   if (!workspace || workspace_bytes < w.bytes) return GRAM_E_WORKSPACE;
+  memset(g_tail_last, 0, sizeof(g_tail_last));
+  if (tail) {
+    const bool on = tail->d_tail >= 2 && tail->d_tail < max_length && tail->sub_rows && K > 1 && !items && !m->long_xattn() &&
+                    tail_shape_ok(B, K, tail->steps) && tail_wanted(m, B, N, L);
+    if (on) {
+      carve_tail(m, workspace, w, B, K, tail->steps);
+      if (workspace_bytes < w.tail_bytes) return GRAM_E_WORKSPACE;
+    } else {
+      tail = nullptr;
+    }
+  }
   w.beam.length_penalty = length_penalty;
-  TRY(generate_body(m, w, input_ids, mask, B, N, L, K, nret, max_length, trie, comp, items, sequences, scores, stream));
+  TRY(generate_body(m, w, input_ids, mask, B, N, L, K, nret, max_length, trie, comp, items, tail, sequences, scores, stream));
   if (width_host) {
     int32_t host[2] = {0, 0};
     hipError_t e = hipMemcpyAsync(&host[0], w.width, sizeof(int32_t), hipMemcpyDeviceToHost, (hipStream_t)stream);
@@ -729,8 +902,23 @@
                                 int nret, int max_length, float length_penalty, const gram_trie_t* trie,
                                 const gram_compaction_t* comp, void* workspace, int64_t workspace_bytes, int64_t* sequences,
                                 float* scores, int32_t* width_host, void* stream) {
-  return generate_call(m, input_ids, mask, B, N, L, K, nret, max_length, length_penalty, trie, comp, nullptr, workspace, workspace_bytes,
-                       sequences, scores, width_host, stream);
+  return generate_call(m, input_ids, mask, B, N, L, K, nret, max_length, length_penalty, trie, comp, nullptr, nullptr, workspace,
+                       workspace_bytes, sequences, scores, width_host, stream);
+}
+
+extern "C" int64_t gram_workspace_bytes_tail(const gram_model_t* m, int B, int N, int L, int K, int max_length, int steps) {
+  if (check_shapes(m, B, N, L, K, max_length) || !tail_shape_ok(B, K, steps)) return GRAM_E_ARG;
+  Workspace w = carve(m, nullptr, B, N, L, K, max_length);
+  carve_tail(m, nullptr, w, B, K, steps);
+  return w.tail_bytes;
+}
+
+extern "C" int gram_generate_tail(const gram_model_t* m, const int64_t* input_ids, const uint8_t* mask, int B, int N, int L, int K,
+                                  int nret, int max_length, float length_penalty, const gram_trie_t* trie,
+                                  const gram_compaction_t* comp, const gram_trie_tail_t* tail, void* workspace,
+                                  int64_t workspace_bytes, int64_t* sequences, float* scores, int32_t* width_host, void* stream) {
+  return generate_call(m, input_ids, mask, B, N, L, K, nret, max_length, length_penalty, trie, comp, nullptr, tail, workspace,
+                       workspace_bytes, sequences, scores, width_host, stream);
 }
 
 extern "C" int gram_generate_items(const gram_model_t* m, const int64_t* input_ids, const uint8_t* mask, int B, int N, int L, int K,
@@ -740,8 +928,8 @@
   if (!items || !items->leaf_lo || !items->leaf_hi || !items->ranks || !items->count || items->stride < 1 ||
       items->stride > GRAM_MAX_USER_ITEMS || (items->mode != GRAM_ITEMS_EXCLUDE && items->mode != GRAM_ITEMS_ALLOW))
     return GRAM_E_ARG;
-  return generate_call(m, input_ids, mask, B, N, L, K, nret, max_length, length_penalty, trie, comp, items, workspace, workspace_bytes,
-                       sequences, scores, width_host, stream);
+  return generate_call(m, input_ids, mask, B, N, L, K, nret, max_length, length_penalty, trie, comp, items, nullptr, workspace,
+                       workspace_bytes, sequences, scores, width_host, stream);
 }
 
 namespace {
diff --git a/gram_amd/model/gram.py b/gram_amd/model/gram.py
--- a/gram_amd/model/gram.py
+++ b/gram_amd/model/gram.py
@@ -142,6 +142,7 @@
         self._packed = None
         self._version = 0
         self._workspace = None
+        self._tail_no_fit = set()
         self._tries: Dict[int, tuple] = {}
         self._precision = os.environ.get("GRAM_PRECISION") or None
         if self._precision is not None and self._precision not in self.PRECISIONS:
@@ -707,6 +708,34 @@
             )
         return self._ensure_workspace(need)
 
+    def _tail_workspace(self, handle, B, N, L, K, max_length, steps) -> Optional[torch.Tensor]:
+        key = (int(handle), B, N, L, K, max_length, steps)
+        if key in self._tail_no_fit:
+            return None
+        dev = self._device()
+        need = int(_lib.load().gram_workspace_bytes_tail(handle, B, N, L, K, max_length, steps))
+        if need <= 0:
+            return None
+        cur = self._workspace if self._workspace is not None and self._workspace.device == dev else None
+        if cur is not None and cur.numel() >= need:
+            return cur
+        free, _total = torch.cuda.mem_get_info(dev)
+        unused = torch.cuda.memory_reserved(dev) - torch.cuda.memory_allocated(dev)
+        room = free + unused + (cur.numel() if cur is not None else 0)
+        if need + self._TAIL_FIT_MARGIN <= room:
+            try:
+                return self._ensure_workspace(need)
+            except torch.cuda.OutOfMemoryError:
+                pass
+        self._tail_no_fit.add(key)
+        import warnings
+        warnings.warn(f"generate: the tail pass needs a workspace of {need / 2**30:.1f} GiB at B={B}, which does not fit this device "
+                      f"next to what it holds; decoding step by step (size the batch with max_users_per_call(..., "
+                      f"prefix_allowed_tokens_fn=fn))")
+        return None
+
+    _TAIL_FIT_MARGIN = 512 * 2**20
+
     def _ensure_workspace(self, need: int) -> torch.Tensor:
         dev = self._device()
         if self._workspace is None or self._workspace.device != dev or self._workspace.numel() < need:
@@ -715,7 +744,22 @@
             self._workspace = torch.empty(int(need), dtype=torch.uint8, device=dev)
         return self._workspace
 
-    def max_users_per_call(self, N: int, L: int, K: int, max_length: int, limit: int = 4096, headroom: float = 0.9) -> int:
+    def _tail_plan(self, fn, K: int, max_length: int, filtered: bool = False):
+        if fn is None or K <= 1 or filtered or self._max_fused_tokens > _lib.GRAM_MAX_FUSED_LEN or self._closure_trie(fn) is None:
+            return 0, 0
+        _sub, d_tail, steps = self._flat_trie(fn).tail_tables()
+        if not (2 <= d_tail < int(max_length) and 1 <= steps <= _lib.GRAM_TAIL_MAX_STEPS):
+            return 0, 0
+        return d_tail, steps
+
+    def _generate_bytes(self, handle, B: int, N: int, Lp: int, K: int, max_length: int, tail_steps: int) -> int:
+        lib = _lib.load()
+        if tail_steps > 0 and lib.gram_tail_pass_wanted(handle, B, N, Lp) == 1:
+            return int(lib.gram_workspace_bytes_tail(handle, B, N, Lp, K, max_length, tail_steps))
+        return int(lib.gram_workspace_bytes(handle, B, N, Lp, K, max_length))
+
+    def max_users_per_call(self, N: int, L: int, K: int, max_length: int, limit: int = 4096, headroom: float = 0.9,
+                           prefix_allowed_tokens_fn: Optional[Callable] = None) -> int:
         self._check_fused_len(N, L)
         handle = self._pack()
         lib = _lib.load()
@@ -727,11 +771,12 @@
             free += self._workspace.numel()
         budget = int(free * headroom)
         lo, hi = 1, max(1, int(limit))
-        if lib.gram_workspace_bytes(handle, hi, N, Lp, K, max_length) <= budget:
+        steps = self._tail_plan(prefix_allowed_tokens_fn, K, max_length)[1]
+        if 0 <= self._generate_bytes(handle, hi, N, Lp, K, max_length, steps) <= budget:
             return hi
         while lo < hi:
             mid = (lo + hi + 1) // 2
-            need = lib.gram_workspace_bytes(handle, mid, N, Lp, K, max_length)
+            need = self._generate_bytes(handle, mid, N, Lp, K, max_length, steps)
             if 0 <= need <= budget:
                 lo = mid
             else:
@@ -970,7 +1015,12 @@
             items = self._user_item_lists(allowed_items if allow else exclude_items, allow, B, flat, candidates, dev)
         comp, harvest_plan = self._plan(ids, mask, B, N, Lp)
         _ctrie, (t_off, t_tok, t_node) = flat.to_device(dev)
-        ws = self._get_workspace(handle, B, N, Lp, K, int(max_length))
+        d_tail, tail_steps = self._tail_plan(prefix_allowed_tokens_fn, K, int(max_length), filtered)
+        tail = tail_steps > 0 and _lib.load().gram_tail_pass_wanted(handle, B, N, Lp) == 1
+        ws = self._tail_workspace(handle, B, N, Lp, K, int(max_length), tail_steps) if tail else None
+        tail = ws is not None
+        if ws is None:
+            ws = self._get_workspace(handle, B, N, Lp, K, int(max_length))
         if K == 1 and nret != 1:
             raise ValueError("num_return_sequences must be 1 for greedy search (num_beams == 1), as in HF generate")
         ct = comp[2] if comp else dict(comp_map=None, comp_ids=None, comp_mask=None, cache_slot=None, cache_x=None, n_cached=0, cache_L=0)
@@ -983,7 +1033,8 @@
             seqs, scores, width = torch.ops.gram.generate_items(*args, leaf_lo, leaf_hi, flat.item_ranks_on(dev, candidates)[1], items,
                                                                 allow)
         else:
-            seqs, scores, width = torch.ops.gram.generate(*args)
+            seqs, scores, width = torch.ops.gram.generate(*args, flat.tail_rows_on(dev) if tail else None, d_tail if tail else 0,
+                                                          tail_steps if tail else 0)
         if harvest_plan is not None:
             self._harvest_from_workspace(harvest_plan, ws, handle, B, N, Lp, K, int(max_length))
         seqs = seqs[:, : int(width[0])]
diff --git a/gram_amd/ops.py b/gram_amd/ops.py
--- a/gram_amd/ops.py
+++ b/gram_amd/ops.py
@@ -37,7 +37,8 @@
              trie_child_tok: Tensor, trie_child_node: Tensor, trie_max_fanout: int, trie_min_seq_len: int, num_beams: int,
              num_return_sequences: int, max_length: int, length_penalty: float, comp_map: Optional[Tensor],
              comp_ids: Optional[Tensor], comp_mask: Optional[Tensor], cache_slot: Optional[Tensor], cache_x: Optional[Tensor],
-             n_cached: int, cache_L: int) -> Tuple[Tensor, Tensor, Tensor]:
+             n_cached: int, cache_L: int, trie_sub_rows: Optional[Tensor] = None, trie_d_tail: int = 0,
+             trie_tail_steps: int = 0) -> Tuple[Tensor, Tensor, Tensor]:
     lib = _lib.load()
     B, N, L = input_ids.shape
     dev = input_ids.device
@@ -51,11 +52,21 @@
     seqs = torch.empty(B * nret, max_length, dtype=torch.int64, device=dev)
     scores = torch.empty(B * nret if K > 1 else 0, dtype=torch.float32, device=dev)
     width = C.c_int32(0)
+    tail = None
+    if trie_sub_rows is not None and trie_d_tail > 0:
+        _check("trie_sub_rows", trie_sub_rows, torch.int32, (trie_child_off.numel() - 1,), dev)
+        tail = _lib.TrieTail(trie_sub_rows.data_ptr(), int(trie_d_tail), int(trie_tail_steps))
     with torch.cuda.device(dev):
-        rc = lib.gram_generate_ex(handle, input_ids.data_ptr(), attention_mask.data_ptr(), B, N, L, K, nret, max_length,
-                                  float(length_penalty), C.byref(trie), C.byref(comp) if comp is not None else None,
-                                  workspace.data_ptr(), workspace.numel(), seqs.data_ptr(), scores.data_ptr() if K > 1 else None,
-                                  C.byref(width), _stream(input_ids))
+        if tail is not None:
+            rc = lib.gram_generate_tail(handle, input_ids.data_ptr(), attention_mask.data_ptr(), B, N, L, K, nret, max_length,
+                                        float(length_penalty), C.byref(trie), C.byref(comp) if comp is not None else None,
+                                        C.byref(tail), workspace.data_ptr(), workspace.numel(), seqs.data_ptr(),
+                                        scores.data_ptr() if K > 1 else None, C.byref(width), _stream(input_ids))
+        else:
+            rc = lib.gram_generate_ex(handle, input_ids.data_ptr(), attention_mask.data_ptr(), B, N, L, K, nret, max_length,
+                                      float(length_penalty), C.byref(trie), C.byref(comp) if comp is not None else None,
+                                      workspace.data_ptr(), workspace.numel(), seqs.data_ptr(), scores.data_ptr() if K > 1 else None,
+                                      C.byref(width), _stream(input_ids))
     _lib.check(rc, "gram_generate")
     return seqs, scores, torch.tensor([width.value], dtype=torch.int32)
 
@@ -63,7 +74,7 @@
 @generate.register_fake
 def _(input_ids, attention_mask, handle, workspace, trie_child_off, trie_child_tok, trie_child_node, trie_max_fanout,
       trie_min_seq_len, num_beams, num_return_sequences, max_length, length_penalty, comp_map, comp_ids, comp_mask, cache_slot,
-      cache_x, n_cached, cache_L):
+      cache_x, n_cached, cache_L, trie_sub_rows=None, trie_d_tail=0, trie_tail_steps=0):
     B = input_ids.shape[0]
     return (input_ids.new_empty(B * num_return_sequences, max_length),
             input_ids.new_empty(B * num_return_sequences if num_beams > 1 else 0, dtype=torch.float32),
diff --git a/gram_amd/runner/base.py b/gram_amd/runner/base.py
--- a/gram_amd/runner/base.py
+++ b/gram_amd/runner/base.py
@@ -145,12 +145,15 @@
         logging.info(f"passage cache: {n} item prompts encoded in {time() - start:.2f}s")
         return n
 
-    def _gpu_batch_users(self, model, n_slots: int, L: int, K: int, max_length: int) -> int:
+    def _gpu_batch_users(self, model, n_slots: int, L: int, K: int, max_length: int, fn=None) -> int:
         explicit = int(_arg(self.args, "eval_gpu_batch", 0) or os.environ.get("GRAM_EVAL_USERS", 0) or 0)
         if explicit > 0:
             return explicit
         if hasattr(model, "max_users_per_call"):
-            return int(model.max_users_per_call(n_slots, L, K, max_length, limit=4096))
+            try:
+                return int(model.max_users_per_call(n_slots, L, K, max_length, limit=4096, prefix_allowed_tokens_fn=fn))
+            except TypeError:
+                return int(model.max_users_per_call(n_slots, L, K, max_length, limit=4096))
         return 4096
 
     def _rescore_unfinished(self, model, input_ids, attention_mask, seqs, scores, fn, K, ref_max_length, shape):
@@ -296,7 +299,7 @@
         collator = getattr(testloader, "collate_fn", None)
         n_slots = int(_arg(self.args, "max_his", 20)) + 1
         L = int(getattr(collator, "item_prompt_max_len", 0) or _arg(self.args, "item_prompt_max_len", 128))
-        users_per_call = self._gpu_batch_users(model, n_slots, L, K, max_length)
+        users_per_call = self._gpu_batch_users(model, n_slots, L, K, max_length, fn)
         lap("candidate_strings")
         logging.info(f"scoring {users_per_call} users per generate() call (--eval_batch_size {_arg(self.args, 'eval_batch_size', 1)} "
                      f"is the loader's; results do not depend on the batch)")
diff --git a/gram_amd/utils/generation_trie.py b/gram_amd/utils/generation_trie.py
--- a/gram_amd/utils/generation_trie.py
+++ b/gram_amd/utils/generation_trie.py
@@ -327,6 +327,60 @@
         self._decoder_rows[int(start_token)] = out
         return out
 
+    TAIL_ROW_FACTOR = 1.10
+
+    def tail_tables(self, factor: Optional[float] = None):
+        f = float(self.TAIL_ROW_FACTOR if factor is None else factor)
+        hit = getattr(self, "_tail_tables", None)
+        if hit is not None and hit[0] == f:
+            return hit[1]
+        from .. import _lib
+
+        n = self.n_nodes
+        fan = np.diff(self.child_off).astype(np.int64)
+        child = self.child_node.astype(np.int64)
+        parent = np.zeros(n, dtype=np.int64)
+        parent[child] = np.repeat(np.arange(n, dtype=np.int64), fan)
+        depth = np.zeros(n, dtype=np.int64)
+        levels, frontier = [], np.zeros(1, dtype=np.int64)
+        while frontier.size:
+            levels.append(frontier)
+            counts = fan[frontier]
+            first = self.child_off[frontier].astype(np.int64)
+            edges = np.repeat(first - (np.cumsum(counts) - counts), counts) + np.arange(int(counts.sum()), dtype=np.int64)
+            frontier = child[edges]
+            depth[frontier] = len(levels)
+        inner = (fan > 0) & (np.arange(n) > 0)
+        sub = inner.astype(np.int64)
+        height = inner.astype(np.int64)
+        for lv in reversed(levels[2:]):
+            np.add.at(sub, parent[lv], sub[lv])
+            np.maximum.at(height, parent[lv], np.where(inner[parent[lv]], height[lv] + 1, 0))
+        sub[~inner] = 0
+        d_tail, steps = 0, 0
+        if inner.any():
+            deepest = int(depth[inner].max())
+            for d in range(deepest, 1, -1):
+                at = inner & (depth == d)
+                if not at.any() or sub[at].sum() > f * height[at].sum():
+                    break
+                if deepest - d + 1 >= 2:
+                    d_tail = d
+            if d_tail and deepest - d_tail + 1 > _lib.GRAM_TAIL_MAX_STEPS:
+                d_tail = 0
+            steps = deepest - d_tail + 1 if d_tail else 0
+        out = (sub.astype(np.int32), int(d_tail), int(steps))
+        self._tail_tables = (f, out)
+        return out
+
+    def tail_rows_on(self, device):
+        import torch
+
+        key = ("tail", str(device))
+        if key not in self._device:
+            self._device[key] = torch.from_numpy(self.tail_tables()[0]).to(device)
+        return self._device[key]
+
     def decoder_rows_on(self, device, start_token: int = 0):
         import torch
 
diff --git a/include/gram_hip.h b/include/gram_hip.h
--- a/include/gram_hip.h
+++ b/include/gram_hip.h
@@ -308,6 +308,44 @@
                         const gram_user_items_t* items_host, void* workspace, int64_t workspace_bytes, int64_t* sequences,
                         float* scores, int32_t* width_host, void* stream);
 
+#define GRAM_TAIL_MAX_STEPS 16
+#define GRAM_TAIL_ENTRY_ROWS 64
+typedef struct {
+  const int32_t* sub_rows;
+  int32_t d_tail;
+  int32_t steps;
+} gram_trie_tail_t;
+typedef struct {
+  int32_t* tokens;
+  int32_t* pos;
+  int32_t* parent;
+  int32_t* root;
+  int32_t* node;
+  int32_t* user_off;
+  int32_t* ent_off;
+  int32_t* ent_users;
+  int32_t* ent_rows;
+  int32_t* rowpos;
+  int32_t* counts;
+  int32_t* slot;
+  int32_t* lvl_rows;
+  int32_t* lvl_tokens;
+  int32_t* lvl_anc;
+  int32_t cap_rows, cap_entries, n_levels, pad_;
+} gram_forest_t;
+int gram_tail_forest(const gram_beam_state_t* st_host, const gram_trie_t* trie_host, const gram_trie_tail_t* tail_host,
+                     const gram_forest_t* forest_host, int t, void* stream);
+int gram_tail_rowpos(const gram_beam_state_t* st_host, const gram_trie_t* trie_host, const gram_forest_t* forest_host, void* stream);
+int gram_scatter_rows(const void* src, const int32_t* rows, void* dst, int n, int row_bytes, int dst_rows, void* stream);
+int gram_cross_attn_entries_split(const void* q, const void* k_layer, const void* vt_layer, const uint8_t* mask, void* out,
+                                  int n_entries, int K, int H, int S, const int32_t* ent_users, const int32_t* ent_rows, int pieces,
+                                  int64_t q_pstride, int64_t bank_pstride, const uint32_t* key_bits, void* stream);
+int64_t gram_workspace_bytes_tail(const gram_model_t* m, int B, int N, int L, int K, int max_length, int steps);
+int gram_generate_tail(const gram_model_t* m, const int64_t* input_ids, const uint8_t* mask, int B, int N, int L, int K, int nret,
+                       int max_length, float length_penalty, const gram_trie_t* trie_host, const gram_compaction_t* compaction_host,
+                       const gram_trie_tail_t* tail_host, void* workspace, int64_t workspace_bytes, int64_t* sequences,
+                       float* scores, int32_t* width_host, void* stream);
+
 int gram_encode_passages(const gram_model_t* m, const int64_t* ids, const uint8_t* mask, int P, int L,
                          void* workspace, int64_t workspace_bytes, float* x_out, void* stream);
 int64_t gram_workspace_encoder_x_offset(const gram_model_t* m, int B, int N, int L, int K, int max_length);
@@ -408,6 +446,13 @@
 
 int gram_debug_set_live_rows(int on);
 int gram_debug_set_token_tables(int on);
+int gram_debug_set_tail_pass(int on);
+int gram_tail_pass_wanted(const gram_model_t* m, int B, int N, int L);
+int gram_debug_set_tail_capacity(int rows);
+int gram_debug_set_tail_level_capacity(int rows);
+int gram_debug_tail_last(int32_t* out4);
+int gram_debug_workspace_beam_state(const gram_model_t* m, void* workspace, int B, int N, int L, int K, int max_length,
+                                    gram_beam_state_t* out);
 int gram_debug_set_beam_chunked(int mode);
 int gram_debug_set_beam_chunk_capacity(int candidates);
 enum gram_stage {
```

Result: faster. 3179 (median of 6 runs) (+1.9%).
